# TorbenHellriegel/Speaker-Recognition-x-vectors

Measured on NVIDIA B200. Metric: x-vectors/sec, higher is better.
Workload: dtype bf16

## Files before the change

include/xvec_b200.h:

```cpp
#ifndef XVEC_B200_H_
#define XVEC_B200_H_

#include <stdint.h>

#ifdef __cplusplus
extern "C" {
#endif

#define XVEC_ABI_VERSION 7

#if defined(__GNUC__)
#define XVEC_API __attribute__((visibility("default")))
#else
#define XVEC_API
#endif

#define XVEC_F32 0
#define XVEC_BF16 1

#define XVEC_OK 0
#define XVEC_E_ARG (-1)
#define XVEC_E_CUDA (-2)
#define XVEC_E_DEVICE (-3)

#define XVEC_MAX_TAPS 8
#define XVEC_TILE_N 256
#define XVEC_POOL_BLOCK 128
#define XVEC_POOL_CHUNK 128
#define XVEC_MAX_STACK 6
#define XVEC_STACK_MAX_BANDS 512
#define XVEC_STACK_MAX_TAP_OFFSET 8

XVEC_API int xvec_abi_version(void);
XVEC_API const char* xvec_last_error(void);
XVEC_API int xvec_device_check(void);
XVEC_API int xvec_watchdog_code(void);
XVEC_API void xvec_watchdog_reset(void);

XVEC_API int xvec_debug_trace(long long* out_host, int n);

XVEC_API int64_t xvec_packed_k(int cin, int taps, int dtype);
XVEC_API int64_t xvec_packed_n(int n);

XVEC_API int xvec_pack_weight(const float* w_dev, int n, int taps, int cin, int dtype, void* out_dev, void* stream);

XVEC_API int xvec_tdnn_layer(const void* x_dev, int x_dtype, int64_t x_rows, int cin, int64_t x_ld,
                    const void* w_packed_dev, int n, const int32_t* tap_offsets_host, int taps,
                    const float* bias_dev, const float* bn_scale_dev, const float* bn_shift_dev, int relu,
                    void* y_dev, int y_dtype, int64_t y_ld, int64_t rows, void* splitk_ws_dev, int64_t splitk_ws_bytes,
                    void* stream);
XVEC_API int64_t xvec_splitk_workspace_bytes(int64_t rows, int cin, int taps, int n, int dtype);

XVEC_API int xvec_tdnn_pool_fused(const void* x_dev, int x_dtype, int64_t x_rows, int cin, int64_t x_ld,
                         const void* w_packed_dev, int n, const int32_t* tap_offsets_host, int taps,
                         const float* bias_dev, const int32_t* row_utt_dev, const int32_t* blk_slot_base_dev,
                         float* part_dev, int64_t rows, void* stream);

XVEC_API int xvec_build_layout(const int32_t* starts_dev, const int32_t* n_pool_dev, const int32_t* slot_start_dev, int n_utts,
                      int64_t rows, int32_t* row_utt_dev, int32_t* blk_slot_base_dev, void* stream);

XVEC_API int xvec_stats_pool_partial(const void* x_dev, int x_dtype, int64_t x_ld, int p, const int64_t* row_start_dev,
                            const int32_t* n_rows_dev, const int32_t* slot_start_dev, int n_utts, int max_chunks,
                            float* part_dev, float* pivot_dev, void* stream);

XVEC_API int xvec_pool_finalize(const float* part_dev, const int32_t* slot_start_dev, const int32_t* n_rows_dev, int n_utts,
                       int p, const float* bn_scale_dev, const float* bn_shift_dev, const float* pivot_dev, float* out_f32_dev,
                       void* out_lp_dev, int out_lp_dtype, int64_t out_lp_ld, void* stream);

typedef struct XvecLayerDesc {
  const void* w_packed_dev;
  const float* bias_dev;
  int32_t n;
  int32_t cin;
  int32_t taps;
  int32_t dtype;
  int32_t tap_offsets[XVEC_MAX_TAPS];
  const void* w_plain_dev;
} XvecLayerDesc;

XVEC_API int64_t xvec_stack_ctrl_bytes(int64_t rows, int n_tdnn);
XVEC_API int64_t xvec_stack_plan(int64_t rows, int n_layers, const int32_t* n_tiles_per_layer_host, int band, uint32_t* items_out_host,
                        int64_t capacity);
XVEC_API int xvec_tdnn_stack(const struct XvecLayerDesc* tdnn_host, int n_tdnn, const void* x_dev, int64_t rows, int64_t x_ld,
                    void* act0_dev, void* act1_dev, int64_t act_ld, const int32_t* row_utt_dev, const int32_t* blk_slot_base_dev,
                    float* part_dev, void* ctrl_dev, int64_t ctrl_bytes, int band, void* stream);

XVEC_API int xvec_linear_small(const void* x_dev, int dtype, int64_t rows, int k, int64_t x_ld, const void* w_dev, int n, int64_t w_ld,
                      const float* bias_dev, int relu, void* y_dev, int y_dtype, int64_t y_ld, void* stream);

XVEC_API int xvec_extract_forward(const XvecLayerDesc* tdnn_host, int n_tdnn, const void* x_dev, int64_t rows, int64_t x_ld,
                         void* act0_dev, void* act1_dev, int64_t act_ld, const int32_t* row_utt_dev,
                         const int32_t* blk_slot_base_dev, const int32_t* utt_slot_start_dev, const int32_t* n_pool_dev,
                         int n_utts, float* part_dev, const float* bn_last_scale_dev, const float* bn_last_shift_dev,
                         float* pooled_dev, void* pooled_lp_dev, const XvecLayerDesc* fc_host, int n_fc, void* fc_tmp_dev,
                         void* splitk_ws_dev, int64_t splitk_ws_bytes, float* out_dev, int64_t out_ld, void* ctrl_dev,
                         int64_t ctrl_bytes, void* stream);

XVEC_API int64_t xvec_mfcc_num_frames(int64_t n_samples);
XVEC_API int xvec_mfcc(const void* wav_dev, int wav_is_int16, const int64_t* wav_start_dev, const int32_t* wav_len_dev,
              const int64_t* row_start_dev, const int32_t* n_frames_dev, int n_utts, int max_frames,
              const float* norm_offset_dev, const float* norm_scale_dev, float* out_dev, int64_t out_ld, void* stream);
XVEC_API int xvec_wav_minmax(const void* wav_dev, int wav_is_int16, const int64_t* wav_start_dev, const int32_t* wav_len_dev,
                    int n_utts, float* norm_offset_dev, float* norm_scale_dev, void* stream);

XVEC_API int xvec_cast(const float* src_dev, int64_t src_ld, void* dst_dev, int dst_dtype, int64_t dst_ld, int64_t rows,
              int cols, void* stream);

XVEC_API int xvec_cosine_trials(const float* xvec_dev, int64_t ld, int dim, const float* mean_dev, const int32_t* enrol_dev,
                       const int32_t* test_dev, int64_t n_trials, float* out_dev, void* stream);

XVEC_API int xvec_split_tf32(const float* x_dev, int64_t ld, int64_t rows, int cols, float* out_dev, int64_t out_ld, void* stream);
XVEC_API int xvec_plda_rowterm(const float* x_dev, int64_t ld, int dim, const float* mean_dev, const float* y_dev, int64_t y_ld,
                      int64_t n, float* q_dev, void* stream);
XVEC_API int xvec_plda_trials(const float* x_dev, int64_t ld, int dim, const float* mean_dev, const float* p_dev, int64_t p_ld,
                     const float* q_dev, const int32_t* enrol_dev, const int32_t* test_dev, int64_t n_trials, float cst, float scale,
                     float* out_dev, void* stream);

#ifdef __cplusplus
}
#endif
#endif
```

speaker-recognition-x-vectors_b200/_lib.py:

```python
from __future__ import annotations

import ctypes
import os
import threading
from ctypes import POINTER, c_char_p, c_float, c_int, c_int32, c_int64, c_void_p

HERE = os.path.dirname(os.path.abspath(__file__))
LIB_PATH = os.environ.get("XVEC_LIB") or os.path.join(HERE, "libxvec_b200.so")

F32, BF16 = 0, 1
E_ARG, E_CUDA, E_DEVICE = -1, -2, -3
TILE_N, POOL_BLOCK, POOL_CHUNK, MAX_TAPS = 256, 128, 128, 8
ABI_VERSION = 7
MAX_STACK = 6
STACK_MAX_TAP_OFFSET = 8

class LayerDesc(ctypes.Structure):
    _fields_ = [("w_packed_dev", c_void_p), ("bias_dev", c_void_p), ("n", c_int32), ("cin", c_int32), ("taps", c_int32),
                ("dtype", c_int32), ("tap_offsets", c_int32 * MAX_TAPS), ("w_plain_dev", c_void_p)]


_SIGNATURES = {
    "xvec_abi_version": (c_int, []),
    "xvec_last_error": (c_char_p, []),
    "xvec_device_check": (c_int, []),
    "xvec_watchdog_code": (c_int, []),
    "xvec_watchdog_reset": (None, []),
    "xvec_debug_trace": (c_int, [c_void_p, c_int]),
    "xvec_packed_k": (c_int64, [c_int, c_int, c_int]),
    "xvec_packed_n": (c_int64, [c_int]),
    "xvec_pack_weight": (c_int, [c_void_p, c_int, c_int, c_int, c_int, c_void_p, c_void_p]),
    "xvec_tdnn_layer": (c_int, [c_void_p, c_int, c_int64, c_int, c_int64, c_void_p, c_int, POINTER(c_int32), c_int,
                                c_void_p, c_void_p, c_void_p, c_int, c_void_p, c_int, c_int64, c_int64, c_void_p, c_int64, c_void_p]),
    "xvec_splitk_workspace_bytes": (c_int64, [c_int64, c_int, c_int, c_int, c_int]),
    "xvec_tdnn_pool_fused": (c_int, [c_void_p, c_int, c_int64, c_int, c_int64, c_void_p, c_int, POINTER(c_int32), c_int,
                                     c_void_p, c_void_p, c_void_p, c_void_p, c_int64, c_void_p]),
    "xvec_build_layout": (c_int, [c_void_p, c_void_p, c_void_p, c_int, c_int64, c_void_p, c_void_p, c_void_p]),
    "xvec_stats_pool_partial": (c_int, [c_void_p, c_int, c_int64, c_int, c_void_p, c_void_p, c_void_p, c_int, c_int,
                                        c_void_p, c_void_p, c_void_p]),
    "xvec_pool_finalize": (c_int, [c_void_p, c_void_p, c_void_p, c_int, c_int, c_void_p, c_void_p, c_void_p, c_void_p, c_void_p,
                                   c_int, c_int64, c_void_p]),
    "xvec_extract_forward": (c_int, [POINTER(LayerDesc), c_int, c_void_p, c_int64, c_int64, c_void_p, c_void_p, c_int64, c_void_p, c_void_p,
                                     c_void_p, c_void_p, c_int, c_void_p, c_void_p, c_void_p, c_void_p, c_void_p, POINTER(LayerDesc), c_int,
                                     c_void_p, c_void_p, c_int64, c_void_p, c_int64, c_void_p, c_int64, c_void_p]),
    "xvec_stack_ctrl_bytes": (c_int64, [c_int64, c_int]),
    "xvec_stack_plan": (c_int64, [c_int64, c_int, POINTER(c_int32), c_int, c_void_p, c_int64]),
    "xvec_linear_small": (c_int, [c_void_p, c_int, c_int64, c_int, c_int64, c_void_p, c_int, c_int64, c_void_p, c_int, c_void_p, c_int, c_int64,
                                  c_void_p]),
    "xvec_tdnn_stack": (c_int, [POINTER(LayerDesc), c_int, c_void_p, c_int64, c_int64, c_void_p, c_void_p, c_int64, c_void_p, c_void_p,
                                c_void_p, c_void_p, c_int64, c_int, c_void_p]),
    "xvec_mfcc_num_frames": (c_int64, [c_int64]),
    "xvec_mfcc": (c_int, [c_void_p, c_int, c_void_p, c_void_p, c_void_p, c_void_p, c_int, c_int, c_void_p, c_void_p, c_void_p, c_int64, c_void_p]),
    "xvec_wav_minmax": (c_int, [c_void_p, c_int, c_void_p, c_void_p, c_int, c_void_p, c_void_p, c_void_p]),
    "xvec_cast": (c_int, [c_void_p, c_int64, c_void_p, c_int, c_int64, c_int64, c_int, c_void_p]),
    "xvec_cosine_trials": (c_int, [c_void_p, c_int64, c_int, c_void_p, c_void_p, c_void_p, c_int64, c_void_p, c_void_p]),
    "xvec_split_tf32": (c_int, [c_void_p, c_int64, c_int64, c_int, c_void_p, c_int64, c_void_p]),
    "xvec_plda_rowterm": (c_int, [c_void_p, c_int64, c_int, c_void_p, c_void_p, c_int64, c_int64, c_void_p, c_void_p]),
    "xvec_plda_trials": (c_int, [c_void_p, c_int64, c_int, c_void_p, c_void_p, c_int64, c_void_p, c_void_p, c_void_p, c_int64, c_float, c_float,
                                 c_void_p, c_void_p]),
}
EXPORTS = tuple(_SIGNATURES)

_lock = threading.Lock()
_lib = None


class XvecError(RuntimeError):
    def __init__(self, code: int, msg: str):
        super().__init__(f"libxvec_b200 error {code}: {msg}")
        self.code = code


def load(build_if_missing: bool = True) -> ctypes.CDLL:
    global _lib
    with _lock:
        if _lib is not None:
            return _lib
        if not os.path.exists(LIB_PATH):
            if not build_if_missing:
                raise ImportError(f"{LIB_PATH} is missing; run speaker-recognition-x-vectors_b200/build.py")
            from . import build as _build
            _build.build()
        lib = ctypes.CDLL(LIB_PATH)
        for name, (res, args) in _SIGNATURES.items():
            fn = getattr(lib, name)
            fn.restype = res
            fn.argtypes = args
        if lib.xvec_abi_version() != ABI_VERSION:
            raise ImportError(f"{LIB_PATH}: ABI {lib.xvec_abi_version()} != expected {ABI_VERSION}; rebuild")
        _lib = lib
        return lib


def check(rc: int) -> None:
    if rc != 0:
        raise XvecError(rc, load().xvec_last_error().decode("utf-8", "replace"))


def ptr(t) -> int | None:
    return None if t is None else t.data_ptr()


def stream_ptr(device_index: int | None = None) -> int:
    import torch
    return torch._C._cuda_getCurrentRawStream(torch.cuda.current_device() if device_index is None else device_index)


class on_device:
    __slots__ = ("ctx",)

    def __init__(self, device):
        import torch
        idx = device.index if device.index is not None else torch.cuda.current_device()
        self.ctx = None if idx == torch.cuda.current_device() else torch.cuda.device(idx)

    def __enter__(self):
        if self.ctx is not None:
            self.ctx.__enter__()

    def __exit__(self, *a):
        if self.ctx is not None:
            return self.ctx.__exit__(*a)


def dtype_code(torch_dtype) -> int:
    import torch
    if torch_dtype == torch.float32:
        return F32
    if torch_dtype == torch.bfloat16:
        return BF16
    raise ValueError(f"unsupported dtype {torch_dtype}; the kernels take float32 (TF32 math) or bfloat16")


def taps_array(offsets):
    arr = (c_int32 * len(offsets))(*[int(o) for o in offsets])
    return arr
```

speaker-recognition-x-vectors_b200/build.py:

```python
from __future__ import annotations

import os
import subprocess
import sys

HERE = os.path.dirname(os.path.abspath(__file__))
CSRC = os.path.join(HERE, "csrc")
LIB = os.path.join(HERE, "libxvec_b200.so")
SOURCES = ["capi.cu", "tdnn_gemm.cu", "tdnn_stack.cu", "fc_small.cu", "pool.cu", "mfcc.cu"]
HEADERS = ["ptx.cuh", "gemm_tile.cuh", "xvec_internal.h", os.path.join("..", "..", "include", "xvec_b200.h")]
NVCC_FLAGS = ["-gencode", "arch=compute_100a,code=sm_100a", "-O3", "-std=c++17", "-lineinfo", "-Xcompiler", "-fPIC",
              "-Xcompiler", "-fvisibility=hidden", "--expt-relaxed-constexpr"]


def _nvcc() -> str:
    for cand in (os.environ.get("NVCC"), "/usr/local/cuda/bin/nvcc", "nvcc"):
        if cand and (os.path.isabs(cand) and os.path.exists(cand) or not os.path.isabs(cand)):
            return cand
    raise RuntimeError("nvcc not found")


DEBUG_LIB = os.path.join(HERE, "libxvec_b200_debug.so")


def needs_build(lib: str = LIB) -> bool:
    if not os.path.exists(lib):
        return True
    t = os.path.getmtime(lib)
    deps = [os.path.join(CSRC, s) for s in SOURCES + HEADERS] + [os.path.abspath(__file__)]
    return any(os.path.getmtime(d) > t for d in deps)


def build(force: bool = False, verbose: bool = False, debug: bool = False) -> str:
    if debug:
        if not force and not needs_build(DEBUG_LIB):
            return DEBUG_LIB
        return _build_to(DEBUG_LIB, list(NVCC_FLAGS) + ["-DXVEC_DEBUG"], verbose, "_dbg")
    if not force and not needs_build():
        return LIB
    return _build_to(LIB, list(NVCC_FLAGS), verbose, "")


def _build_to(lib: str, flags, verbose: bool, suffix: str) -> str:
    flags = flags + (["-Xptxas", "-v"] if verbose else [])
    objs = []
    for s in SOURCES:
        obj = os.path.join(CSRC, s.replace(".cu", suffix + ".o"))
        cmd = [_nvcc()] + flags + ["-c", os.path.join(CSRC, s), "-o", obj]
        r = subprocess.run(cmd, capture_output=True, text=True)
        if verbose or r.returncode:
            sys.stderr.write(r.stdout + r.stderr)
        if r.returncode:
            raise RuntimeError(f"nvcc failed on {s}")
        objs.append(obj)
    cmd = [_nvcc(), "-shared", "-o", lib] + objs + ["-lcudart"]
    r = subprocess.run(cmd, capture_output=True, text=True)
    if r.returncode:
        sys.stderr.write(r.stdout + r.stderr)
        raise RuntimeError("link failed")
    return lib


if __name__ == "__main__":
    print(build(force="--force" in sys.argv, verbose="--verbose" in sys.argv, debug="--debug" in sys.argv))
```

speaker-recognition-x-vectors_b200/csrc/capi.cu:

```cuda
#include <stdarg.h>
#include <stdio.h>

#include "xvec_internal.h"

namespace xvec {

static thread_local char g_err[512] = "";

int set_error(int code, const char* fmt, ...) {
  va_list ap;
  va_start(ap, fmt);
  vsnprintf(g_err, sizeof(g_err), fmt, ap);
  va_end(ap);
  return code;
}

namespace {
struct DevInfo {
  int checked = 0;
  int sms = 0;
  int major = 0, minor = 0;
};
DevInfo g_dev[64];

DevInfo* cur_dev() {
  int d = 0;
  if (cudaGetDevice(&d) != cudaSuccess || d < 0 || d >= 64) return nullptr;
  DevInfo* di = &g_dev[d];
  if (!di->checked) {
    cudaDeviceProp prop;
    if (cudaGetDeviceProperties(&prop, d) != cudaSuccess) return nullptr;
    di->sms = prop.multiProcessorCount;
    di->major = prop.major;
    di->minor = prop.minor;
    di->checked = (prop.major == 10) ? 1 : -1;
  }
  return di;
}
}

int device_check() {
  DevInfo* di = cur_dev();
  if (!di) return set_error(XVEC_E_CUDA, "no usable CUDA device: %s", cudaGetErrorString(cudaGetLastError()));
  if (di->checked < 0)
    return set_error(XVEC_E_DEVICE, "device is sm_%d%d; these kernels are built for sm_100a only (no fallback)", di->major, di->minor);
  return XVEC_OK;
}

int num_sms() {
  DevInfo* di = cur_dev();
  return di ? di->sms : 1;
}

PFN_encodeTiled get_encode_tiled() {
  static const PFN_encodeTiled fn = [] {
    void* p = nullptr;
    cudaDriverEntryPointQueryResult qres;
    if (cudaGetDriverEntryPoint("cuTensorMapEncodeTiled", &p, cudaEnableDefault, &qres) == cudaSuccess &&
        qres == cudaDriverEntryPointSuccess)
      return reinterpret_cast<PFN_encodeTiled>(p);
    return static_cast<PFN_encodeTiled>(nullptr);
  }();
  return fn;
}

unsigned int* watchdog_host_word() {
  static std::mutex mu;
  static unsigned int* word = nullptr;
  std::lock_guard<std::mutex> lock(mu);
  if (!word) {
    void* p = nullptr;
    if (cudaHostAlloc(&p, 64, cudaHostAllocMapped | cudaHostAllocPortable) != cudaSuccess) return nullptr;
    word = static_cast<unsigned int*>(p);
    *word = 0u;
  }
  return word;
}

int read_watchdog() {
  unsigned int* w = watchdog_host_word();
  return w ? static_cast<int>(*reinterpret_cast<volatile unsigned int*>(w)) : 0;
}

int layer_desc(XvecLayerDesc* l, const void* w_packed, const float* bias, int n, int cin, int taps, int dtype, const int32_t* tap_offsets) {
  if (!tap_offsets) return set_error(XVEC_E_ARG, "tap_offsets_host is NULL");
  if (taps < 1 || taps > XVEC_MAX_TAPS) return set_error(XVEC_E_ARG, "taps must be in [1,%d]", XVEC_MAX_TAPS);
  *l = XvecLayerDesc{};
  l->w_packed_dev = w_packed;
  l->bias_dev = bias;
  l->n = n;
  l->cin = cin;
  l->taps = taps;
  l->dtype = dtype;
  for (int j = 0; j < taps; ++j) l->tap_offsets[j] = tap_offsets[j];
  return XVEC_OK;
}

}

using namespace xvec;

extern "C" {

int xvec_abi_version(void) { return XVEC_ABI_VERSION; }
const char* xvec_last_error(void) { return g_err; }
int xvec_device_check(void) { return device_check(); }
int xvec_watchdog_code(void) {
  cudaDeviceSynchronize();
  return read_watchdog();
}
void xvec_watchdog_reset(void) {
  if (unsigned int* w = watchdog_host_word()) *reinterpret_cast<volatile unsigned int*>(w) = 0u;
}

int xvec_debug_trace(long long* out_host, int n) { return read_trace(out_host, n); }

int64_t xvec_packed_k(int cin, int taps, int dtype) {
  const int kc = chunk_elems(dtype);
  return static_cast<int64_t>(taps) * ((cin + kc - 1) / kc) * kc;
}
int64_t xvec_splitk_workspace_bytes(int64_t rows, int cin, int taps, int n, int dtype) {
  if (rows <= 0 || cin <= 0 || taps < 1 || n <= 0) return 0;
  return splitk_workspace_bytes(rows, cin, taps, n, dtype);
}
int64_t xvec_packed_n(int n) { return static_cast<int64_t>((n + XVEC_TILE_N - 1) / XVEC_TILE_N) * XVEC_TILE_N; }

int xvec_tdnn_layer(const void* x_dev, int x_dtype, int64_t x_rows, int cin, int64_t x_ld, const void* w_packed_dev, int n,
                    const int32_t* tap_offsets_host, int taps, const float* bias_dev, const float* bn_scale_dev,
                    const float* bn_shift_dev, int relu, void* y_dev, int y_dtype, int64_t y_ld, int64_t rows, void* splitk_ws_dev,
                    int64_t splitk_ws_bytes, void* stream) {
  XvecLayerDesc l;
  const int rc = layer_desc(&l, w_packed_dev, bias_dev, n, cin, taps, x_dtype, tap_offsets_host);
  if (rc) return rc;
  return gemm_store(l, x_dev, x_rows, x_ld, rows, bn_scale_dev, bn_shift_dev, relu, y_dev, y_dtype, y_ld, splitk_ws_dev, splitk_ws_bytes,
                    stream);
}

int xvec_tdnn_pool_fused(const void* x_dev, int x_dtype, int64_t x_rows, int cin, int64_t x_ld, const void* w_packed_dev, int n,
                         const int32_t* tap_offsets_host, int taps, const float* bias_dev, const int32_t* row_utt_dev,
                         const int32_t* blk_slot_base_dev, float* part_dev, int64_t rows, void* stream) {
  XvecLayerDesc l;
  const int rc = layer_desc(&l, w_packed_dev, bias_dev, n, cin, taps, x_dtype, tap_offsets_host);
  if (rc) return rc;
  return gemm_pool(l, x_dev, x_rows, x_ld, rows, row_utt_dev, blk_slot_base_dev, part_dev, stream);
}

int64_t xvec_stack_ctrl_bytes(int64_t rows, int n_tdnn) { return stack_ctrl_bytes(rows, n_tdnn); }
int64_t xvec_stack_plan(int64_t rows, int n_layers, const int32_t* n_tiles_per_layer_host, int band, uint32_t* items_out_host,
                        int64_t capacity) {
  return stack_plan(rows, n_layers, n_tiles_per_layer_host, band, items_out_host, capacity);
}

int xvec_linear_small(const void* x_dev, int dtype, int64_t rows, int k, int64_t x_ld, const void* w_dev, int n, int64_t w_ld,
                      const float* bias_dev, int relu, void* y_dev, int y_dtype, int64_t y_ld, void* stream) {
  return fc_small_dispatch(x_dev, dtype, rows, k, x_ld, w_dev, n, w_ld, bias_dev, relu, y_dev, y_dtype, y_ld, stream);
}

int xvec_tdnn_stack(const XvecLayerDesc* tdnn, int n_tdnn, const void* x_dev, int64_t rows, int64_t x_ld, void* act0_dev, void* act1_dev,
                    int64_t act_ld, const int32_t* row_utt_dev, const int32_t* blk_slot_base_dev, float* part_dev, void* ctrl_dev,
                    int64_t ctrl_bytes, int band, void* stream) {
  if (!tdnn) return set_error(XVEC_E_ARG, "tdnn_host is NULL");
  return stack_dispatch(tdnn, n_tdnn, x_dev, rows, x_ld, act0_dev, act1_dev, act_ld, row_utt_dev, blk_slot_base_dev, part_dev, ctrl_dev,
                        ctrl_bytes, band, stream);
}

static int frame_stack(const XvecLayerDesc* tdnn, int n_tdnn, const void* x, int64_t rows, int64_t x_ld, void* act0, void* act1,
                       int64_t act_ld, const int32_t* row_utt, const int32_t* blk_slot_base, float* part, void* ctrl, int64_t ctrl_bytes,
                       void* stream) {
  if (ctrl && stack_supported(tdnn, n_tdnn, rows))
    return stack_dispatch(tdnn, n_tdnn, x, rows, x_ld, act0, act1, act_ld, row_utt, blk_slot_base, part, ctrl, ctrl_bytes, 0, stream);
  void* act[2] = {act0, act1};
  const void* h = x;
  int64_t h_ld = x_ld;
  for (int i = 0; i + 1 < n_tdnn; ++i) {
    const int rc = gemm_store(tdnn[i], h, rows, h_ld, rows, nullptr, nullptr, 1, act[i & 1], tdnn[i + 1].dtype, act_ld, nullptr, 0, stream);
    if (rc) return rc;
    h = act[i & 1];
    h_ld = act_ld;
  }
  return gemm_pool(tdnn[n_tdnn - 1], h, rows, h_ld, rows, row_utt, blk_slot_base, part, stream);
}

static int segment_head(const XvecLayerDesc* fc, int n_fc, const void* a, int64_t a_ld, int n_utts, void* fc_tmp, void* splitk_ws,
                        int64_t splitk_ws_bytes, float* out, int64_t out_ld, void* stream) {
  for (int i = 0; i < n_fc; ++i) {
    const XvecLayerDesc& l = fc[i];
    const bool final_layer = i == n_fc - 1;
    void* y = final_layer ? static_cast<void*>(out) : fc_tmp;
    const int y_dtype = final_layer ? XVEC_F32 : fc[i + 1].dtype;
    const int64_t y_ld = final_layer ? out_ld : l.n;
    const int relu = final_layer ? 0 : 1;
    int rc;
    if (l.w_plain_dev && fc_small_supported(n_utts, l.cin, l.n, a_ld, l.cin, a, l.w_plain_dev, l.dtype))
      rc = fc_small_dispatch(a, l.dtype, n_utts, l.cin, a_ld, l.w_plain_dev, l.n, l.cin, l.bias_dev, relu, y, y_dtype, y_ld, stream);
    else
      rc = gemm_store(l, a, n_utts, a_ld, n_utts, nullptr, nullptr, relu, y, y_dtype, y_ld, splitk_ws, splitk_ws_bytes, stream);
    if (rc) return rc;
    a = y;
    a_ld = y_ld;
  }
  return XVEC_OK;
}

int xvec_extract_forward(const XvecLayerDesc* tdnn, int n_tdnn, const void* x_dev, int64_t rows, int64_t x_ld, void* act0_dev,
                         void* act1_dev, int64_t act_ld, const int32_t* row_utt_dev, const int32_t* blk_slot_base_dev,
                         const int32_t* utt_slot_start_dev, const int32_t* n_pool_dev, int n_utts, float* part_dev,
                         const float* bn_last_scale_dev, const float* bn_last_shift_dev, float* pooled_dev, void* pooled_lp_dev,
                         const XvecLayerDesc* fc, int n_fc, void* fc_tmp_dev, void* splitk_ws_dev, int64_t splitk_ws_bytes,
                         float* out_dev, int64_t out_ld, void* ctrl_dev, int64_t ctrl_bytes, void* stream) {
  if (!tdnn || n_tdnn < 2 || n_fc < 0 || n_fc > 2 || (n_fc > 0 && !fc))
    return set_error(XVEC_E_ARG, "need >= 2 TDNN layers and 0 to 2 segment layers");
  if (!x_dev || !act0_dev || !act1_dev || !pooled_dev || (n_fc > 0 && !out_dev)) return set_error(XVEC_E_ARG, "null pointer argument");
  if (n_fc == 2 && !fc_tmp_dev) return set_error(XVEC_E_ARG, "fc_tmp_dev is NULL");
  const bool lp_head = n_fc > 0 && fc[0].dtype == XVEC_BF16;
  if (lp_head && !pooled_lp_dev) return set_error(XVEC_E_ARG, "pooled_lp_dev is required for bf16 segment layers");
  int rc = frame_stack(tdnn, n_tdnn, x_dev, rows, x_ld, act0_dev, act1_dev, act_ld, row_utt_dev, blk_slot_base_dev, part_dev, ctrl_dev,
                       ctrl_bytes, stream);
  if (rc) return rc;
  const int64_t pooled_ld = 2 * static_cast<int64_t>(tdnn[n_tdnn - 1].n);
  rc = xvec_pool_finalize(part_dev, utt_slot_start_dev, n_pool_dev, n_utts, tdnn[n_tdnn - 1].n, bn_last_scale_dev, bn_last_shift_dev, nullptr,
                          pooled_dev, pooled_lp_dev, XVEC_BF16, pooled_ld, stream);
  if (rc) return rc;
  return segment_head(fc, n_fc, lp_head ? pooled_lp_dev : static_cast<const void*>(pooled_dev), pooled_ld, n_utts, fc_tmp_dev, splitk_ws_dev,
                      splitk_ws_bytes, out_dev, out_ld, stream);
}

}
```

speaker-recognition-x-vectors_b200/csrc/pool.cu:

```cuda
#include <cuda_bf16.h>

#include "xvec_internal.h"

namespace xvec {

template <bool kBf16>
__global__ void __launch_bounds__(128)
stats_pool_partial_kernel(const void* __restrict__ x, long long ld, int p, const long long* __restrict__ row_start,
                          const int* __restrict__ n_rows, const int* __restrict__ slot_start, float* __restrict__ part,
                          float* __restrict__ pivot_out) {
  const int u = blockIdx.x;
  const int nr = n_rows[u];
  const int r0 = blockIdx.y * XVEC_POOL_CHUNK;
  if (r0 >= nr) return;
  const int r1 = min(nr, r0 + XVEC_POOL_CHUNK);
  const int c = (blockIdx.z * 128 + threadIdx.x) * 4;
  if (c >= p) return;
  const long long first = row_start[u] + r0;
  float s0 = 0.f, s1 = 0.f, s2 = 0.f, s3 = 0.f, q0 = 0.f, q1 = 0.f, q2 = 0.f, q3 = 0.f;
  float4 pv = make_float4(0.f, 0.f, 0.f, 0.f);
  auto acc = [&](float a, float b, float cc, float d) {
    a -= pv.x; b -= pv.y; cc -= pv.z; d -= pv.w;
    s0 += a; s1 += b; s2 += cc; s3 += d;
    q0 = fmaf(a, a, q0); q1 = fmaf(b, b, q1); q2 = fmaf(cc, cc, q2); q3 = fmaf(d, d, q3);
  };
  constexpr int U = 8;
  int r = r0;
  if constexpr (kBf16) {
    const uint2* src = reinterpret_cast<const uint2*>(reinterpret_cast<const __nv_bfloat16*>(x) + first * ld + c);
    const long long step = ld / 4;
    if (pivot_out) {
      const uint2 w = __ldg(reinterpret_cast<const uint2*>(reinterpret_cast<const __nv_bfloat16*>(x) + row_start[u] * ld + c));
      const float2 a = __bfloat1622float2(*reinterpret_cast<const __nv_bfloat162*>(&w.x));
      const float2 b = __bfloat1622float2(*reinterpret_cast<const __nv_bfloat162*>(&w.y));
      pv = make_float4(a.x, a.y, b.x, b.y);
    }
    for (; r + U <= r1; r += U) {
      uint2 v[U];
#pragma unroll
      for (int i = 0; i < U; ++i) v[i] = __ldcs(src + static_cast<long long>(r - r0 + i) * step);
#pragma unroll
      for (int i = 0; i < U; ++i) {
        const float2 a = __bfloat1622float2(*reinterpret_cast<const __nv_bfloat162*>(&v[i].x));
        const float2 b = __bfloat1622float2(*reinterpret_cast<const __nv_bfloat162*>(&v[i].y));
        acc(a.x, a.y, b.x, b.y);
      }
    }
    for (; r < r1; ++r) {
      const uint2 w = __ldcs(src + static_cast<long long>(r - r0) * step);
      const float2 a = __bfloat1622float2(*reinterpret_cast<const __nv_bfloat162*>(&w.x));
      const float2 b = __bfloat1622float2(*reinterpret_cast<const __nv_bfloat162*>(&w.y));
      acc(a.x, a.y, b.x, b.y);
    }
  } else {
    const float4* src = reinterpret_cast<const float4*>(reinterpret_cast<const float*>(x) + first * ld + c);
    const long long step = ld / 4;
    if (pivot_out) pv = __ldg(reinterpret_cast<const float4*>(reinterpret_cast<const float*>(x) + row_start[u] * ld + c));
    for (; r + U <= r1; r += U) {
      float4 v[U];
#pragma unroll
      for (int i = 0; i < U; ++i) v[i] = __ldcs(src + static_cast<long long>(r - r0 + i) * step);
#pragma unroll
      for (int i = 0; i < U; ++i) acc(v[i].x, v[i].y, v[i].z, v[i].w);
    }
    for (; r < r1; ++r) {
      const float4 w = __ldcs(src + static_cast<long long>(r - r0) * step);
      acc(w.x, w.y, w.z, w.w);
    }
  }
  if (pivot_out && blockIdx.y == 0) *reinterpret_cast<float4*>(pivot_out + static_cast<size_t>(u) * p + c) = pv;
  float* dst = part + static_cast<size_t>(slot_start[u] + blockIdx.y) * 2 * p + c;
  *reinterpret_cast<float4*>(dst) = make_float4(s0, s1, s2, s3);
  *reinterpret_cast<float4*>(dst + p) = make_float4(q0, q1, q2, q3);
}

__global__ void __launch_bounds__(128)
pool_finalize_kernel(const float* __restrict__ part, const int* __restrict__ slot_start, const int* __restrict__ n_rows, int p,
                     const float* __restrict__ scale, const float* __restrict__ shift, const float* __restrict__ pivot,
                     float* __restrict__ out, void* __restrict__ out_lp, int lp_dtype, long long lp_ld) {
  const int u = blockIdx.x;
  const int col = blockIdx.y * 128 + threadIdx.x;
  __shared__ double inv_n[2];
  if (threadIdx.x == 0) {
    const int n0 = n_rows[u];
    inv_n[0] = n0 > 0 ? 1.0 / n0 : 0.0;
    inv_n[1] = n0 > 1 ? 1.0 / (n0 - 1) : 0.0;
  }
  __syncthreads();
  if (col >= p) return;
  const int sl0 = slot_start[u], sl1 = slot_start[u + 1];
  double S = 0.0, Q = 0.0;
  int sl = sl0;
  for (; sl + 4 <= sl1; sl += 4) {
    float a[4], b[4];
#pragma unroll
    for (int i = 0; i < 4; ++i) {
      const float* src = part + static_cast<size_t>(sl + i) * 2 * p + col;
      a[i] = src[0];
      b[i] = src[p];
    }
#pragma unroll
    for (int i = 0; i < 4; ++i) {
      S += static_cast<double>(a[i]);
      Q += static_cast<double>(b[i]);
    }
  }
  for (; sl < sl1; ++sl) {
    const float* src = part + static_cast<size_t>(sl) * 2 * p + col;
    S += static_cast<double>(src[0]);
    Q += static_cast<double>(src[p]);
  }
  const int n = n_rows[u];
  const double nan = __longlong_as_double(0x7ff8000000000000LL);
  const double mean = n > 0 ? S * inv_n[0] + (pivot ? static_cast<double>(pivot[static_cast<size_t>(u) * p + col]) : 0.0) : nan;
  double var = n > 1 ? (Q - S * S * inv_n[0]) * inv_n[1] : nan;
  if (var < 0.0) var = 0.0;
  const float sc = scale ? scale[col] : 1.f;
  const float sh = shift ? shift[col] : 0.f;
  const float m = static_cast<float>(mean * sc + sh);
  const float sd = fabsf(sc) * sqrtf(static_cast<float>(var));
  out[static_cast<size_t>(u) * 2 * p + col] = m;
  out[static_cast<size_t>(u) * 2 * p + p + col] = sd;
  if (out_lp) {
    if (lp_dtype == XVEC_BF16) {
      __nv_bfloat16* o = reinterpret_cast<__nv_bfloat16*>(out_lp) + static_cast<size_t>(u) * lp_ld;
      o[col] = __float2bfloat16_rn(m);
      o[p + col] = __float2bfloat16_rn(sd);
    } else {
      float* o = reinterpret_cast<float*>(out_lp) + static_cast<size_t>(u) * lp_ld;
      o[col] = m;
      o[p + col] = sd;
    }
  }
}

__global__ void __launch_bounds__(256)
build_layout_kernel(const int* __restrict__ starts, const int* __restrict__ n_pool, const int* __restrict__ slot_start, int n_utts,
                    int rows, int n_blocks, int* __restrict__ row_utt, int* __restrict__ blk_slot_base) {
  const int i = blockIdx.x * blockDim.x + threadIdx.x;
  if (i < rows) {
    int lo = 0, hi = n_utts - 1;
    while (lo < hi) {
      const int mid = (lo + hi + 1) >> 1;
      if (starts[mid] <= i) lo = mid; else hi = mid - 1;
    }
    row_utt[i] = (i - starts[lo] < n_pool[lo]) ? lo : -1;
  }
  if (i < n_blocks) {
    const int first_row = i * XVEC_POOL_BLOCK;
    int lo = 0, hi = n_utts;
    while (lo < hi) {
      const int mid = (lo + hi) >> 1;
      if (starts[mid] + n_pool[mid] - 1 >= first_row) hi = mid; else lo = mid + 1;
    }
    int base = 0;
    if (lo < n_utts) {
      const int b0 = starts[lo] / XVEC_POOL_BLOCK;
      base = slot_start[lo] + (i > b0 ? i - b0 : 0);
    }
    blk_slot_base[i] = base;
  }
}

__global__ void cast_kernel(const float* __restrict__ src, long long src_ld, void* __restrict__ dst, int dst_dtype, long long dst_ld,
                            long long rows, int cols) {
  const long long total = rows * cols;
  for (long long i = blockIdx.x * static_cast<long long>(blockDim.x) + threadIdx.x; i < total;
       i += static_cast<long long>(gridDim.x) * blockDim.x) {
    const long long r = i / cols;
    const int c = static_cast<int>(i - r * cols);
    const float v = src[r * src_ld + c];
    if (dst_dtype == XVEC_BF16)
      reinterpret_cast<__nv_bfloat16*>(dst)[r * dst_ld + c] = __float2bfloat16_rn(v);
    else
      reinterpret_cast<float*>(dst)[r * dst_ld + c] = v;
  }
}

__global__ void pack_weight_kernel(const float* __restrict__ w, int n, int taps, int cin, int tap_k, long long n_pad, long long k_pad,
                                   int dtype, void* __restrict__ out) {
  const long long total = n_pad * k_pad;
  for (long long i = blockIdx.x * static_cast<long long>(blockDim.x) + threadIdx.x; i < total;
       i += static_cast<long long>(gridDim.x) * blockDim.x) {
    const long long row = i / k_pad;
    const int kk = static_cast<int>(i - row * k_pad);
    const int tap = kk / tap_k;
    const int ch = kk - tap * tap_k;
    const float v = (row < n && ch < cin) ? w[row * (static_cast<long long>(taps) * cin) + tap * cin + ch] : 0.f;
    const int bke = dtype == XVEC_BF16 ? 64 : 32;
    const long long o = (static_cast<long long>(kk / bke) * n_pad + row) * bke + kk % bke;
    if (dtype == XVEC_BF16)
      reinterpret_cast<__nv_bfloat16*>(out)[o] = __float2bfloat16_rn(v);
    else
      reinterpret_cast<float*>(out)[o] = v;
  }
}

__global__ void __launch_bounds__(256)
cosine_trials_kernel(const float* __restrict__ xv, long long ld, int dim, const float* __restrict__ mean, const int* __restrict__ enrol,
                     const int* __restrict__ test, long long n_trials, float* __restrict__ out) {
  const long long t = (blockIdx.x * static_cast<long long>(blockDim.x) + threadIdx.x) >> 5;
  const int lane = threadIdx.x & 31;
  if (t >= n_trials) return;
  const float* a = xv + static_cast<long long>(enrol[t]) * ld;
  const float* b = xv + static_cast<long long>(test[t]) * ld;
  float ab = 0.f, aa = 0.f, bb = 0.f;
  for (int i = lane; i < dim; i += 32) {
    const float mu = mean ? mean[i] : 0.f;
    const float x = a[i] - mu, y = b[i] - mu;
    ab = fmaf(x, y, ab);
    aa = fmaf(x, x, aa);
    bb = fmaf(y, y, bb);
  }
#pragma unroll
  for (int o = 16; o > 0; o >>= 1) {
    ab += __shfl_xor_sync(0xffffffffu, ab, o);
    aa += __shfl_xor_sync(0xffffffffu, aa, o);
    bb += __shfl_xor_sync(0xffffffffu, bb, o);
  }
  if (lane == 0) out[t] = ab * rsqrtf(aa) * rsqrtf(bb);
}

__global__ void split_tf32_kernel(const float* __restrict__ x, long long ld, long long rows, int cols, float* __restrict__ out, long long out_ld) {
  const long long total = rows * cols;
  for (long long i = blockIdx.x * static_cast<long long>(blockDim.x) + threadIdx.x; i < total;
       i += static_cast<long long>(gridDim.x) * blockDim.x) {
    const long long r = i / cols;
    const int c = static_cast<int>(i - r * cols);
    const float v = x[r * ld + c];
    const float hi = __uint_as_float(__float_as_uint(v) & 0xFFFFE000u);
    float* o = out + r * out_ld + c;
    o[0] = hi;
    o[cols] = v - hi;
    o[2 * cols] = hi;
  }
}
__global__ void __launch_bounds__(256)
plda_rowterm_kernel(const float* __restrict__ x, long long ld, int dim, const float* __restrict__ mean, const float* __restrict__ y,
                    long long y_ld, long long n, float* __restrict__ q) {
  const long long r = (blockIdx.x * static_cast<long long>(blockDim.x) + threadIdx.x) >> 5;
  const int lane = threadIdx.x & 31;
  if (r >= n) return;
  float acc = 0.f;
  for (int i = lane; i < dim; i += 32) acc = fmaf(x[r * ld + i] - mean[i], y[r * y_ld + i], acc);
#pragma unroll
  for (int o = 16; o > 0; o >>= 1) acc += __shfl_xor_sync(0xffffffffu, acc, o);
  if (lane == 0) q[r] = 0.5f * acc;
}
__global__ void __launch_bounds__(256)
plda_trials_kernel(const float* __restrict__ x, long long ld, int dim, const float* __restrict__ mean, const float* __restrict__ p,
                   long long p_ld, const float* __restrict__ q, const int* __restrict__ enrol, const int* __restrict__ test,
                   long long n_trials, float cst, float scale, float* __restrict__ out) {
  const long long t = (blockIdx.x * static_cast<long long>(blockDim.x) + threadIdx.x) >> 5;
  const int lane = threadIdx.x & 31;
  if (t >= n_trials) return;
  const int e = enrol[t], s = test[t];
  const float* pe = p + static_cast<long long>(e) * p_ld;
  const float* xs = x + static_cast<long long>(s) * ld;
  float acc = 0.f;
  for (int i = lane; i < dim; i += 32) acc = fmaf(pe[i], xs[i] - mean[i], acc);
#pragma unroll
  for (int o = 16; o > 0; o >>= 1) acc += __shfl_xor_sync(0xffffffffu, acc, o);
  if (lane == 0) out[t] = scale * (q[e] + q[s] + acc + cst);
}

static int grid_for(long long total) {
  const long long want = (total + 255) / 256;
  const long long cap = static_cast<long long>(num_sms()) * 16;
  return static_cast<int>(want < cap ? want : cap);
}

static int check_launch(const char* what) {
  cudaError_t e = cudaGetLastError();
  if (e != cudaSuccess) return set_error(XVEC_E_CUDA, "%s launch: %s", what, cudaGetErrorString(e));
  return XVEC_OK;
}

}

using namespace xvec;

extern "C" {

int xvec_build_layout(const int32_t* starts_dev, const int32_t* n_pool_dev, const int32_t* slot_start_dev, int n_utts, int64_t rows,
                      int32_t* row_utt_dev, int32_t* blk_slot_base_dev, void* stream) {
  int rc = device_check();
  if (rc) return rc;
  if (!starts_dev || !n_pool_dev || !slot_start_dev || !row_utt_dev || !blk_slot_base_dev) return set_error(XVEC_E_ARG, "null pointer argument");
  if (n_utts <= 0 || rows <= 0 || rows > 0x7fffff00LL) return set_error(XVEC_E_ARG, "bad n_utts / rows");
  const int n_blocks = static_cast<int>((rows + 255) / 256) * (256 / XVEC_POOL_BLOCK);
  const long long n = rows > n_blocks ? rows : n_blocks;
  build_layout_kernel<<<static_cast<unsigned>((n + 255) / 256), 256, 0, static_cast<cudaStream_t>(stream)>>>(
      starts_dev, n_pool_dev, slot_start_dev, n_utts, static_cast<int>(rows), n_blocks, row_utt_dev, blk_slot_base_dev);
  return check_launch("build_layout_kernel");
}

int xvec_stats_pool_partial(const void* x_dev, int x_dtype, int64_t x_ld, int p, const int64_t* row_start_dev,
                            const int32_t* n_rows_dev, const int32_t* slot_start_dev, int n_utts, int max_chunks, float* part_dev,
                            float* pivot_dev, void* stream) {
  int rc = device_check();
  if (rc) return rc;
  if (!x_dev || !row_start_dev || !n_rows_dev || !slot_start_dev || !part_dev) return set_error(XVEC_E_ARG, "null pointer argument");
  if (x_dtype != XVEC_F32 && x_dtype != XVEC_BF16) return set_error(XVEC_E_ARG, "bad x_dtype %d", x_dtype);
  if (p <= 0 || p % 4 != 0 || x_ld % 4 != 0 || x_ld < p) return set_error(XVEC_E_ARG, "p and x_ld must be positive multiples of 4, x_ld >= p");
  const int align = x_dtype == XVEC_BF16 ? 8 : 16;
  if ((reinterpret_cast<uintptr_t>(x_dev) % align) != 0 || (reinterpret_cast<uintptr_t>(part_dev) & 15u) != 0 ||
      (reinterpret_cast<uintptr_t>(pivot_dev) & 15u) != 0)
    return set_error(XVEC_E_ARG, "x_dev / part_dev / pivot_dev are not sufficiently aligned");
  if (n_utts <= 0 || max_chunks <= 0 || max_chunks > 65535) return set_error(XVEC_E_ARG, "bad n_utts / max_chunks");
  dim3 grid(n_utts, max_chunks, (p + 511) / 512);
  cudaStream_t st = static_cast<cudaStream_t>(stream);
  if (x_dtype == XVEC_BF16)
    stats_pool_partial_kernel<true><<<grid, 128, 0, st>>>(x_dev, x_ld, p, reinterpret_cast<const long long*>(row_start_dev), n_rows_dev,
                                                         slot_start_dev, part_dev, pivot_dev);
  else
    stats_pool_partial_kernel<false><<<grid, 128, 0, st>>>(x_dev, x_ld, p, reinterpret_cast<const long long*>(row_start_dev), n_rows_dev,
                                                          slot_start_dev, part_dev, pivot_dev);
  return check_launch("stats_pool_partial_kernel");
}

int xvec_pool_finalize(const float* part_dev, const int32_t* slot_start_dev, const int32_t* n_rows_dev, int n_utts, int p,
                       const float* bn_scale_dev, const float* bn_shift_dev, const float* pivot_dev, float* out_f32_dev, void* out_lp_dev,
                       int out_lp_dtype, int64_t out_lp_ld, void* stream) {
  int rc = device_check();
  if (rc) return rc;
  if (!part_dev || !slot_start_dev || !n_rows_dev || !out_f32_dev) return set_error(XVEC_E_ARG, "null pointer argument");
  if (n_utts <= 0 || p <= 0) return set_error(XVEC_E_ARG, "non-positive size");
  if ((bn_scale_dev == nullptr) != (bn_shift_dev == nullptr)) return set_error(XVEC_E_ARG, "bn_scale and bn_shift must be given together");
  if (out_lp_dev && (out_lp_dtype != XVEC_F32 && out_lp_dtype != XVEC_BF16)) return set_error(XVEC_E_ARG, "bad out_lp_dtype");
  if (out_lp_dev && out_lp_ld < 2 * p) return set_error(XVEC_E_ARG, "out_lp_ld < 2p");
  dim3 grid(n_utts, (p + 127) / 128);
  pool_finalize_kernel<<<grid, 128, 0, static_cast<cudaStream_t>(stream)>>>(part_dev, slot_start_dev, n_rows_dev, p, bn_scale_dev,
                                                                            bn_shift_dev, pivot_dev, out_f32_dev, out_lp_dev, out_lp_dtype,
                                                                            out_lp_ld);
  return check_launch("pool_finalize_kernel");
}

int xvec_cast(const float* src_dev, int64_t src_ld, void* dst_dev, int dst_dtype, int64_t dst_ld, int64_t rows, int cols, void* stream) {
  int rc = device_check();
  if (rc) return rc;
  if (!src_dev || !dst_dev) return set_error(XVEC_E_ARG, "null pointer argument");
  if (rows <= 0 || cols <= 0 || src_ld < cols || dst_ld < cols) return set_error(XVEC_E_ARG, "bad shape");
  if (dst_dtype != XVEC_F32 && dst_dtype != XVEC_BF16) return set_error(XVEC_E_ARG, "bad dst_dtype");
  const long long total = rows * cols;
  const int blocks = grid_for(total);
  cast_kernel<<<blocks, 256, 0, static_cast<cudaStream_t>(stream)>>>(src_dev, src_ld, dst_dev, dst_dtype, dst_ld, rows, cols);
  return check_launch("cast_kernel");
}

int xvec_pack_weight(const float* w_dev, int n, int taps, int cin, int dtype, void* out_dev, void* stream) {
  int rc = device_check();
  if (rc) return rc;
  if (!w_dev || !out_dev) return set_error(XVEC_E_ARG, "null pointer argument");
  if (n <= 0 || cin <= 0 || taps < 1 || taps > XVEC_MAX_TAPS) return set_error(XVEC_E_ARG, "bad shape");
  if (dtype != XVEC_F32 && dtype != XVEC_BF16) return set_error(XVEC_E_ARG, "bad dtype");
  const long long k_pad = xvec_packed_k(cin, taps, dtype);
  const long long n_pad = xvec_packed_n(n);
  const long long total = n_pad * k_pad;
  const int blocks = grid_for(total);
  pack_weight_kernel<<<blocks, 256, 0, static_cast<cudaStream_t>(stream)>>>(w_dev, n, taps, cin, static_cast<int>(k_pad / taps), n_pad,
                                                                           k_pad, dtype, out_dev);
  return check_launch("pack_weight_kernel");
}

int xvec_cosine_trials(const float* xvec_dev, int64_t ld, int dim, const float* mean_dev, const int32_t* enrol_dev,
                       const int32_t* test_dev, int64_t n_trials, float* out_dev, void* stream) {
  int rc = device_check();
  if (rc) return rc;
  if (!xvec_dev || !enrol_dev || !test_dev || !out_dev) return set_error(XVEC_E_ARG, "null pointer argument");
  if (dim <= 0 || ld < dim || n_trials <= 0) return set_error(XVEC_E_ARG, "bad shape");
  const long long blocks = (n_trials * 32 + 255) / 256;
  cosine_trials_kernel<<<static_cast<unsigned>(blocks), 256, 0, static_cast<cudaStream_t>(stream)>>>(xvec_dev, ld, dim, mean_dev, enrol_dev,
                                                                                                   test_dev, n_trials, out_dev);
  return check_launch("cosine_trials_kernel");
}

int xvec_split_tf32(const float* x_dev, int64_t ld, int64_t rows, int cols, float* out_dev, int64_t out_ld, void* stream) {
  int rc = device_check();
  if (rc) return rc;
  if (!x_dev || !out_dev) return set_error(XVEC_E_ARG, "null pointer argument");
  if (rows <= 0 || cols <= 0 || ld < cols || out_ld < 3 * static_cast<int64_t>(cols)) return set_error(XVEC_E_ARG, "bad shape");
  split_tf32_kernel<<<grid_for(rows * cols), 256, 0, static_cast<cudaStream_t>(stream)>>>(x_dev, ld, rows, cols, out_dev, out_ld);
  return check_launch("split_tf32_kernel");
}

int xvec_plda_rowterm(const float* x_dev, int64_t ld, int dim, const float* mean_dev, const float* y_dev, int64_t y_ld, int64_t n,
                      float* q_dev, void* stream) {
  int rc = device_check();
  if (rc) return rc;
  if (!x_dev || !mean_dev || !y_dev || !q_dev) return set_error(XVEC_E_ARG, "null pointer argument");
  if (dim <= 0 || ld < dim || y_ld < dim || n <= 0) return set_error(XVEC_E_ARG, "bad shape");
  const long long blocks = (n * 32 + 255) / 256;
  plda_rowterm_kernel<<<static_cast<unsigned>(blocks), 256, 0, static_cast<cudaStream_t>(stream)>>>(x_dev, ld, dim, mean_dev, y_dev, y_ld, n, q_dev);
  return check_launch("plda_rowterm_kernel");
}

int xvec_plda_trials(const float* x_dev, int64_t ld, int dim, const float* mean_dev, const float* p_dev, int64_t p_ld, const float* q_dev,
                     const int32_t* enrol_dev, const int32_t* test_dev, int64_t n_trials, float cst, float scale, float* out_dev,
                     void* stream) {
  int rc = device_check();
  if (rc) return rc;
  if (!x_dev || !mean_dev || !p_dev || !q_dev || !enrol_dev || !test_dev || !out_dev) return set_error(XVEC_E_ARG, "null pointer argument");
  if (dim <= 0 || ld < dim || p_ld < dim || n_trials <= 0) return set_error(XVEC_E_ARG, "bad shape");
  const long long blocks = (n_trials * 32 + 255) / 256;
  plda_trials_kernel<<<static_cast<unsigned>(blocks), 256, 0, static_cast<cudaStream_t>(stream)>>>(x_dev, ld, dim, mean_dev, p_dev, p_ld, q_dev,
                                                                                                 enrol_dev, test_dev, n_trials, cst, scale, out_dev);
  return check_launch("plda_trials_kernel");
}

}
```

speaker-recognition-x-vectors_b200/csrc/ptx.cuh:

```cuda
#pragma once
#include <cuda_runtime.h>
#include <cuda.h>
#include <stdint.h>

namespace xvec {

static __device__ unsigned int* g_watchdog_ptr = nullptr;

static __device__ __noinline__ void watchdog_report(unsigned int code) {
  unsigned int* p = g_watchdog_ptr;
  if (p) {
    *reinterpret_cast<volatile unsigned int*>(p) = code;
    __threadfence_system();
  }
}
static __device__ __noinline__ void watchdog_trip(unsigned int code) {
  watchdog_report(code);
  __trap();
}

__device__ __forceinline__ uint32_t smem_u32(const void* p) {
  return static_cast<uint32_t>(__cvta_generic_to_shared(p));
}

__device__ __forceinline__ bool elect_one() {
  uint32_t pred;
  asm volatile("{\n\t.reg .pred p;\n\telect.sync _|p, 0xffffffff;\n\tselp.u32 %0, 1, 0, p;\n\t}" : "=r"(pred));
  return pred != 0;
}

__device__ __forceinline__ void mbar_init(uint64_t* bar, uint32_t count) {
  asm volatile("mbarrier.init.shared::cta.b64 [%0], %1;" ::"r"(smem_u32(bar)), "r"(count) : "memory");
}
__device__ __forceinline__ void fence_mbar_init() {
  asm volatile("fence.mbarrier_init.release.cluster;" ::: "memory");
}
__device__ __forceinline__ void mbar_expect_tx(uint64_t* bar, uint32_t bytes) {
  asm volatile("mbarrier.arrive.expect_tx.shared::cta.b64 _, [%0], %1;" ::"r"(smem_u32(bar)), "r"(bytes) : "memory");
}
__device__ __forceinline__ void mbar_arrive(uint64_t* bar) {
  asm volatile("mbarrier.arrive.shared::cta.b64 _, [%0];" ::"r"(smem_u32(bar)) : "memory");
}
__device__ __forceinline__ bool mbar_try_wait(uint64_t* bar, uint32_t parity) {
  uint32_t done;
  asm volatile(
      "{\n\t.reg .pred p;\n\t"
      "mbarrier.try_wait.parity.shared::cta.b64 p, [%1], %2;\n\t"
      "selp.u32 %0, 1, 0, p;\n\t}"
      : "=r"(done)
      : "r"(smem_u32(bar)), "r"(parity)
      : "memory");
  return done != 0;
}
__device__ __forceinline__ bool mbar_test_wait(uint64_t* bar, uint32_t parity) {
  uint32_t done;
  asm volatile(
      "{\n\t.reg .pred p;\n\t"
      "mbarrier.test_wait.parity.shared::cta.b64 p, [%1], %2;\n\t"
      "selp.u32 %0, 1, 0, p;\n\t}"
      : "=r"(done)
      : "r"(smem_u32(bar)), "r"(parity)
      : "memory");
  return done != 0;
}
__device__ __forceinline__ void mbar_wait(uint64_t* bar, uint32_t parity, uint32_t code) {
  uint32_t spins = 0;
  while (!mbar_try_wait(bar, parity)) {
    if (++spins > (1u << 26)) {
      watchdog_trip(code);
    }
  }
}

__device__ __forceinline__ bool mbar_try_wait_a(uint32_t bar_addr, uint32_t parity) {
  uint32_t done;
  asm volatile(
      "{\n\t.reg .pred p;\n\t"
      "mbarrier.try_wait.parity.shared::cta.b64 p, [%1], %2;\n\t"
      "selp.u32 %0, 1, 0, p;\n\t}"
      : "=r"(done)
      : "r"(bar_addr), "r"(parity)
      : "memory");
  return done != 0;
}
__device__ __forceinline__ void mbar_wait_a(uint32_t bar_addr, uint32_t parity, uint32_t code) {
  uint32_t spins = 0;
  while (!mbar_try_wait_a(bar_addr, parity)) {
    if (++spins > (1u << 26)) watchdog_trip(code);
  }
}
__device__ __forceinline__ void mbar_expect_tx_a(uint32_t bar_addr, uint32_t bytes) {
  asm volatile("mbarrier.arrive.expect_tx.shared::cta.b64 _, [%0], %1;" ::"r"(bar_addr), "r"(bytes) : "memory");
}

__device__ __forceinline__ uint32_t mapa_u32(uint32_t smem_addr, uint32_t cta_rank) {
  uint32_t r;
  asm volatile("mapa.shared::cluster.u32 %0, %1, %2;" : "=r"(r) : "r"(smem_addr), "r"(cta_rank));
  return r;
}
__device__ __forceinline__ void mbar_arrive_cluster(uint32_t cluster_addr) {
  asm volatile("mbarrier.arrive.shared::cluster.b64 _, [%0];" ::"r"(cluster_addr) : "memory");
}
__device__ __forceinline__ uint32_t cluster_ctarank() {
  uint32_t r;
  asm volatile("mov.u32 %0, %%cluster_ctarank;" : "=r"(r));
  return r;
}
__device__ __forceinline__ void cluster_sync_all() {
  asm volatile("barrier.cluster.arrive.release.aligned;" ::: "memory");
  asm volatile("barrier.cluster.wait.acquire.aligned;" ::: "memory");
}

__device__ __forceinline__ void mbar_arrive_expect_tx_cluster(uint32_t cluster_addr, uint32_t bytes) {
  asm volatile("mbarrier.arrive.expect_tx.shared::cluster.b64 _, [%0], %1;" ::"r"(cluster_addr), "r"(bytes) : "memory");
}
__device__ __forceinline__ void st_async_cluster_u32(uint32_t cluster_addr, uint32_t v, uint32_t cluster_mbar) {
  asm volatile("st.async.weak.shared::cluster.mbarrier::complete_tx::bytes.u32 [%0], %1, [%2];" ::"r"(cluster_addr), "r"(v), "r"(cluster_mbar) : "memory");
}

__device__ __forceinline__ uint32_t ld_acquire_gpu_u32(const uint32_t* p) {
  uint32_t v;
  asm volatile("ld.acquire.gpu.global.u32 %0, [%1];" : "=r"(v) : "l"(p) : "memory");
  return v;
}
__device__ __forceinline__ void red_release_gpu_add_u32(uint32_t* p, uint32_t v) {
  asm volatile("red.release.gpu.global.add.u32 [%0], %1;" ::"l"(p), "r"(v) : "memory");
}
__device__ __forceinline__ uint32_t atom_add_acq_rel_cta_shared_u32(uint32_t smem_addr, uint32_t v) {
  uint32_t old;
  asm volatile("atom.acq_rel.cta.shared::cta.add.u32 %0, [%1], %2;" : "=r"(old) : "r"(smem_addr), "r"(v) : "memory");
  return old;
}
__device__ __forceinline__ void fence_proxy_async_global() { asm volatile("fence.proxy.async.global;" ::: "memory"); }

__device__ __forceinline__ void fence_proxy_async_smem() {
  asm volatile("fence.proxy.async.shared::cta;" ::: "memory");
}
__device__ __forceinline__ void tc_fence_before() { asm volatile("tcgen05.fence::before_thread_sync;" ::: "memory"); }
__device__ __forceinline__ void tc_fence_after() { asm volatile("tcgen05.fence::after_thread_sync;" ::: "memory"); }

__device__ __forceinline__ void tma_prefetch_desc(const CUtensorMap* m) {
  asm volatile("prefetch.tensormap [%0];" ::"l"(reinterpret_cast<uint64_t>(m)) : "memory");
}
__device__ __forceinline__ void tma_store_2d(const CUtensorMap* m, const void* smem_src, int32_t c0, int32_t c1, uint64_t l2_policy) {
  asm volatile("cp.async.bulk.tensor.2d.global.shared::cta.bulk_group.L2::cache_hint [%0, {%2, %3}], [%1], %4;"
               ::"l"(reinterpret_cast<uint64_t>(m)), "r"(smem_u32(smem_src)), "r"(c0), "r"(c1), "l"(l2_policy)
               : "memory");
}
constexpr uint64_t L2_EVICT_NORMAL = 0x1000000000000000ull;
constexpr uint64_t L2_EVICT_FIRST = 0x12F0000000000000ull;
constexpr uint64_t L2_EVICT_LAST = 0x14F0000000000000ull;
__device__ __forceinline__ void tma_store_commit() { asm volatile("cp.async.bulk.commit_group;" ::: "memory"); }
template <int kPending>
__device__ __forceinline__ void tma_store_wait_read() {
  asm volatile("cp.async.bulk.wait_group.read %0;" ::"n"(kPending) : "memory");
}
__device__ __forceinline__ void tma_store_wait_all() { asm volatile("cp.async.bulk.wait_group 0;" ::: "memory"); }
template <int kPending>
__device__ __forceinline__ void tma_store_wait_done() {
  asm volatile("cp.async.bulk.wait_group %0;" ::"n"(kPending) : "memory");
}

template <uint32_t kCols>
__device__ __forceinline__ void tmem_alloc_pair(uint32_t* smem_result) {
  asm volatile("tcgen05.alloc.cta_group::2.sync.aligned.shared::cta.b32 [%0], %1;" ::"r"(smem_u32(smem_result)), "n"(kCols) : "memory");
  asm volatile("tcgen05.relinquish_alloc_permit.cta_group::2.sync.aligned;" ::: "memory");
}
template <uint32_t kCols>
__device__ __forceinline__ void tmem_dealloc_pair(uint32_t taddr) {
  asm volatile("tcgen05.dealloc.cta_group::2.sync.aligned.b32 %0, %1;" ::"r"(taddr), "n"(kCols) : "memory");
}

__device__ __forceinline__ uint64_t umma_desc_sw128(uint32_t smem_addr) {
  return static_cast<uint64_t>((smem_addr & 0x3FFFFu) >> 4) | (1ull << 16) | (static_cast<uint64_t>(1024 >> 4) << 32) |
         (1ull << 46) | (2ull << 61);
}

__host__ __device__ constexpr uint32_t umma_idesc(uint32_t fmt, uint32_t m, uint32_t n) {
  return (1u << 4) | (fmt << 7) | (fmt << 10) | ((n >> 3) << 17) | ((m >> 4) << 24);
}

__device__ __forceinline__ uint32_t tma_step_pair(uint32_t elected, uint32_t is_leader, uint32_t full_bar_local, uint32_t full_bar_leader,
                                                  uint32_t tx_bytes, uint32_t smem_a, const CUtensorMap* map_a, int32_t a0, int32_t a1,
                                                  uint64_t pol_a, uint32_t smem_b, const CUtensorMap* map_b, int32_t b0, int32_t b1,
                                                  uint64_t pol_b, uint32_t probe_bar, uint32_t probe_par) {
  uint32_t rdy;
  asm volatile(
      "{\n\t"
      ".reg .pred pe, pl, pw;\n\t"
      "setp.ne.b32 pe, %1, 0;\n\t"
      "setp.ne.b32 pl, %2, 0;\n\t"
      "and.pred pl, pl, pe;\n\t"
      "@pl mbarrier.arrive.expect_tx.shared::cta.b64 _, [%3], %5;\n\t"
      "@pe cp.async.bulk.tensor.2d.cta_group::2.shared::cluster.global.mbarrier::complete_tx::bytes.L2::cache_hint [%6], [%7, {%8, %9}], [%4], %10;\n\t"
      "@pe cp.async.bulk.tensor.2d.cta_group::2.shared::cluster.global.mbarrier::complete_tx::bytes.L2::cache_hint [%11], [%12, {%13, %14}], [%4], %17;\n\t"
      "mbarrier.try_wait.parity.shared::cta.b64 pw, [%15], %16;\n\t"
      "selp.u32 %0, 1, 0, pw;\n\t"
      "}"
      : "=r"(rdy)
      : "r"(elected), "r"(is_leader), "r"(full_bar_local), "r"(full_bar_leader), "r"(tx_bytes), "r"(smem_a),
        "l"(reinterpret_cast<uint64_t>(map_a)), "r"(a0), "r"(a1), "l"(pol_a), "r"(smem_b), "l"(reinterpret_cast<uint64_t>(map_b)),
        "r"(b0), "r"(b1), "r"(probe_bar), "r"(probe_par), "l"(pol_b)
      : "memory");
  return rdy;
}

__device__ __forceinline__ uint32_t tma_step_one(uint32_t elected, uint32_t is_leader, uint32_t do_load, uint32_t bar_local, uint32_t bar_leader,
                                                 uint32_t tx, uint32_t smem_dst, const CUtensorMap* map, int32_t c0, int32_t c1, uint64_t pol,
                                                 uint32_t probe_bar, uint32_t probe_par) {
  uint32_t rdy;
  asm volatile(
      "{\n\t"
      ".reg .pred pe, pl, pw;\n\t"
      "setp.ne.b32 pe, %1, 0;\n\t"
      "setp.ne.b32 pl, %2, 0;\n\t"
      "and.pred pl, pl, pe;\n\t"
      "mbarrier.test_wait.parity.shared::cta.b64 pw, [%11], %12;\n\t"
      "@pl mbarrier.arrive.expect_tx.shared::cta.b64 _, [%3], %5;\n\t"
      "@pe cp.async.bulk.tensor.2d.cta_group::2.shared::cluster.global.mbarrier::complete_tx::bytes.L2::cache_hint [%6], [%7, {%8, %9}], [%4], %10;\n\t"
      "selp.u32 %0, 1, 0, pw;\n\t"
      "}"
      : "=r"(rdy)
      : "r"(elected & do_load), "r"(is_leader), "r"(bar_local), "r"(bar_leader), "r"(tx), "r"(smem_dst), "l"(reinterpret_cast<uint64_t>(map)),
        "r"(c0), "r"(c1), "l"(pol), "r"(probe_bar), "r"(probe_par)
      : "memory");
  return rdy;
}

__device__ __forceinline__ void tma_load_2d_pair(uint32_t bar_leader, uint32_t smem_dst, const CUtensorMap* map, int32_t c0, int32_t c1, uint64_t pol) {
  asm volatile(
      "cp.async.bulk.tensor.2d.cta_group::2.shared::cluster.global.mbarrier::complete_tx::bytes.L2::cache_hint [%0], [%1, {%2, %3}], [%4], %5;"
      ::"r"(smem_dst), "l"(reinterpret_cast<uint64_t>(map)), "r"(c0), "r"(c1), "r"(bar_leader), "l"(pol)
      : "memory");
}

enum { STEP_COMMIT_A = 1, STEP_COMMIT_B = 2, STEP_PROBE_A = 4, STEP_PROBE_B = 8 };
template <bool kTf32>
__device__ __forceinline__ uint32_t umma_step_pair(uint32_t elected, uint32_t tmem_d, uint64_t da, uint64_t db, uint32_t idesc,
                                                   uint32_t acc0, uint32_t flags, uint32_t commit_a_bar, uint32_t commit_b_bar,
                                                   uint32_t probe_a_bar, uint32_t probe_a_par, uint32_t probe_b_bar,
                                                   uint32_t probe_b_par) {
  uint32_t rdy;
#define XVEC_STEP_BODY(KIND)                                                                                      \
  asm volatile(                                                                                                   \
      "{\n\t"                                                                                                     \
      ".reg .pred pe, pacc, pt, pca, pcb, ppa, ppb, pwa, pwb;\n\t"                                                \
      ".reg .b64 a1, a2, a3, b1, b2, b3;\n\t"                                                                     \
      ".reg .b32 ra, rb, f;\n\t"                                                                                  \
      ".reg .b16 mk;\n\t"                                                                                         \
      "mov.b16 mk, 3;\n\t"                                                                                        \
      "setp.ne.b32 pe, %1, 0;\n\t"                                                                                \
      "setp.ne.b32 pacc, %6, 0;\n\t"                                                                              \
      "setp.eq.b32 pt, 0, 0;\n\t"                                                                                 \
      "and.b32 f, %7, 4;\n\tsetp.ne.b32 ppa, f, 0;\n\t"                                                          \
      "and.b32 f, %7, 8;\n\tsetp.ne.b32 ppb, f, 0;\n\t"                                                          \
      "setp.ne.b32 pwa, 0, 0;\n\t"                                                                                \
      "setp.ne.b32 pwb, 0, 0;\n\t"                                                                                \
      "@ppa mbarrier.test_wait.parity.shared::cta.b64 pwa, [%10], %11;\n\t"                                       \
      "@ppb mbarrier.test_wait.parity.shared::cta.b64 pwb, [%12], %13;\n\t"                                       \
      "add.u64 a1, %3, 2;\n\tadd.u64 a2, %3, 4;\n\tadd.u64 a3, %3, 6;\n\t"                                      \
      "add.u64 b1, %4, 2;\n\tadd.u64 b2, %4, 4;\n\tadd.u64 b3, %4, 6;\n\t"                                      \
      "@pe tcgen05.mma.cta_group::2.kind::" KIND " [%2], %3, %4, %5, pacc;\n\t"                                   \
      "@pe tcgen05.mma.cta_group::2.kind::" KIND " [%2], a1, b1, %5, pt;\n\t"                                     \
      "@pe tcgen05.mma.cta_group::2.kind::" KIND " [%2], a2, b2, %5, pt;\n\t"                                     \
      "@pe tcgen05.mma.cta_group::2.kind::" KIND " [%2], a3, b3, %5, pt;\n\t"                                     \
      "and.b32 f, %7, 2;\n\tsetp.ne.b32 pcb, f, 0;\n\tand.pred pcb, pcb, pe;\n\t"                               \
      "and.b32 f, %7, 1;\n\tsetp.ne.b32 pca, f, 0;\n\tand.pred pca, pca, pe;\n\t"                               \
      "@pcb tcgen05.commit.cta_group::2.mbarrier::arrive::one.shared::cluster.multicast::cluster.b64 [%9], mk;\n\t" \
      "@pca tcgen05.commit.cta_group::2.mbarrier::arrive::one.shared::cluster.multicast::cluster.b64 [%8], mk;\n\t" \
      "selp.u32 ra, 1, 0, pwa;\n\t"                                                                               \
      "selp.u32 rb, 2, 0, pwb;\n\t"                                                                               \
      "or.b32 %0, ra, rb;\n\t"                                                                                    \
      "}"                                                                                                         \
      : "=r"(rdy)                                                                                                 \
      : "r"(elected), "r"(tmem_d), "l"(da), "l"(db), "r"(idesc), "r"(acc0), "r"(flags), "r"(commit_a_bar),        \
        "r"(commit_b_bar), "r"(probe_a_bar), "r"(probe_a_par), "r"(probe_b_bar), "r"(probe_b_par)                 \
      : "memory")
  if constexpr (kTf32) {
    XVEC_STEP_BODY("tf32");
  } else {
    XVEC_STEP_BODY("f16");
  }
#undef XVEC_STEP_BODY
  return rdy;
}
template <bool kTf32, bool kLastTap>
__device__ __forceinline__ uint32_t umma_step_fixed(uint32_t elected, uint32_t tmem_d, uint32_t a_lo, uint32_t b_lo, uint32_t desc_hi, uint32_t idesc,
                                                    uint32_t acc0, uint32_t commit_a_bar, uint32_t commit_b_bar, uint32_t probe_a_bar,
                                                    uint32_t probe_a_par, uint32_t probe_b_bar, uint32_t probe_b_par) {
  uint32_t rdy;
#define XVEC_FIXED_BODY(KIND, PROBE_A, COMMIT_A)                                                                  \
  asm volatile(                                                                                                   \
      "{\n\t"                                                                                                     \
      ".reg .pred pe, pacc, pt, pwa, pwb;\n\t"                                                                    \
      ".reg .b64 a0, a1, a2, a3, b0, b1, b2, b3;\n\t"                                                             \
      ".reg .b32 ra, rb, t;\n\t"                                                                                  \
      ".reg .b16 mk;\n\t"                                                                                         \
      "mov.b16 mk, 3;\n\t"                                                                                        \
      "setp.ne.b32 pe, %13, 0;\n\t"                                                                               \
      "setp.ne.b32 pacc, %6, 0;\n\t"                                                                              \
      "setp.eq.b32 pt, 0, 0;\n\t"                                                                                 \
      "setp.ne.b32 pwa, 0, 0;\n\t"                                                                                \
      PROBE_A                                                                                                     \
      "mbarrier.test_wait.parity.shared::cta.b64 pwb, [%11], %12;\n\t"                                            \
      "mov.b64 a0, {%2, %4};\n\t"                                                                                 \
      "mov.b64 b0, {%3, %4};\n\t"                                                                                 \
      "add.u32 t, %2, 2;\n\tmov.b64 a1, {t, %4};\n\t"                                                            \
      "add.u32 t, %3, 2;\n\tmov.b64 b1, {t, %4};\n\t"                                                            \
      "add.u32 t, %2, 4;\n\tmov.b64 a2, {t, %4};\n\t"                                                            \
      "add.u32 t, %3, 4;\n\tmov.b64 b2, {t, %4};\n\t"                                                            \
      "add.u32 t, %2, 6;\n\tmov.b64 a3, {t, %4};\n\t"                                                            \
      "add.u32 t, %3, 6;\n\tmov.b64 b3, {t, %4};\n\t"                                                            \
      "@pe tcgen05.mma.cta_group::2.kind::" KIND " [%1], a0, b0, %5, pacc;\n\t"                                   \
      "@pe tcgen05.mma.cta_group::2.kind::" KIND " [%1], a1, b1, %5, pt;\n\t"                                     \
      "@pe tcgen05.mma.cta_group::2.kind::" KIND " [%1], a2, b2, %5, pt;\n\t"                                     \
      "@pe tcgen05.mma.cta_group::2.kind::" KIND " [%1], a3, b3, %5, pt;\n\t"                                     \
      "@pe tcgen05.commit.cta_group::2.mbarrier::arrive::one.shared::cluster.multicast::cluster.b64 [%8], mk;\n\t" \
      COMMIT_A                                                                                                    \
      "selp.u32 ra, 1, 0, pwa;\n\t"                                                                               \
      "selp.u32 rb, 2, 0, pwb;\n\t"                                                                               \
      "or.b32 %0, ra, rb;\n\t"                                                                                    \
      "}"                                                                                                         \
      : "=r"(rdy)                                                                                                 \
      : "r"(tmem_d), "r"(a_lo), "r"(b_lo), "r"(desc_hi), "r"(idesc), "r"(acc0), "r"(commit_a_bar), "r"(commit_b_bar),  \
        "r"(probe_a_bar), "r"(probe_a_par), "r"(probe_b_bar), "r"(probe_b_par), "r"(elected)                      \
      : "memory")
#define XVEC_FIXED_PROBE_A "mbarrier.test_wait.parity.shared::cta.b64 pwa, [%9], %10;\n\t"
#define XVEC_FIXED_COMMIT_A "@pe tcgen05.commit.cta_group::2.mbarrier::arrive::one.shared::cluster.multicast::cluster.b64 [%7], mk;\n\t"
  if constexpr (kTf32) {
    if constexpr (kLastTap) XVEC_FIXED_BODY("tf32", XVEC_FIXED_PROBE_A, XVEC_FIXED_COMMIT_A);
    else XVEC_FIXED_BODY("tf32", "", "");
  } else {
    if constexpr (kLastTap) XVEC_FIXED_BODY("f16", XVEC_FIXED_PROBE_A, XVEC_FIXED_COMMIT_A);
    else XVEC_FIXED_BODY("f16", "", "");
  }
#undef XVEC_FIXED_BODY
#undef XVEC_FIXED_PROBE_A
#undef XVEC_FIXED_COMMIT_A
  return rdy;
}
__device__ __forceinline__ void umma_commit_pair(uint64_t* bar, uint16_t cta_mask) {
  asm volatile("tcgen05.commit.cta_group::2.mbarrier::arrive::one.shared::cluster.multicast::cluster.b64 [%0], %1;"
               ::"r"(smem_u32(bar)), "h"(cta_mask) : "memory");
}
__device__ __forceinline__ void tmem_ld_32x32(uint32_t taddr, uint32_t (&v)[32]) {
  asm volatile(
      "tcgen05.ld.sync.aligned.32x32b.x32.b32 "
      "{%0, %1, %2, %3, %4, %5, %6, %7, %8, %9, %10, %11, %12, %13, %14, %15, "
      "%16, %17, %18, %19, %20, %21, %22, %23, %24, %25, %26, %27, %28, %29, %30, %31}, [%32];"
      : "=r"(v[0]), "=r"(v[1]), "=r"(v[2]), "=r"(v[3]), "=r"(v[4]), "=r"(v[5]), "=r"(v[6]), "=r"(v[7]), "=r"(v[8]),
        "=r"(v[9]), "=r"(v[10]), "=r"(v[11]), "=r"(v[12]), "=r"(v[13]), "=r"(v[14]), "=r"(v[15]), "=r"(v[16]),
        "=r"(v[17]), "=r"(v[18]), "=r"(v[19]), "=r"(v[20]), "=r"(v[21]), "=r"(v[22]), "=r"(v[23]), "=r"(v[24]),
        "=r"(v[25]), "=r"(v[26]), "=r"(v[27]), "=r"(v[28]), "=r"(v[29]), "=r"(v[30]), "=r"(v[31])
      : "r"(taddr)
      : "memory");
}
__device__ __forceinline__ void tmem_ld_wait() { asm volatile("tcgen05.wait::ld.sync.aligned;" ::: "memory"); }

}
```

speaker-recognition-x-vectors_b200/csrc/tdnn_stack.cu:

```cuda
#include "gemm_tile.cuh"
#include <cuda_bf16.h>

#include <mutex>
#include <type_traits>

namespace xvec {

template <bool kAllTf32>
struct StackCfg {
  static constexpr int SLOTS = 10;
  static constexpr int BOX_W = kAllTf32 ? 128 : 64;
  static constexpr int BOX_BYTES = 32 * BOX_W;
  static constexpr int NBUF = kAllTf32 ? 1 : 2;
  static constexpr int STAGE_BYTES = NBUF * BOX_BYTES;
};
constexpr int SLAB_ROWS_MAX = BM_CTA + XVEC_STACK_MAX_TAP_OFFSET;
constexpr int SLAB_BYTES = SLAB_ROWS_MAX * BK_BYTES;
constexpr int SLOT_BYTES = SLAB_BYTES;
static_assert(SLOT_BYTES % 1024 == 0 && SLOT_BYTES >= B_BYTES, "slot bases must stay 1024-byte aligned for SWIZZLE_128B and hold a weight tile");
constexpr int SCHED_SLOTS = 8;
constexpr int CREDIT_BARS = 4;
constexpr int STACK_RUNAHEAD = 1;
constexpr uint32_t ITEM_DONE = 0xFFFFFFFFu;
constexpr int SCHED_CONSUMERS = 2 * EPI_WARPS + 6;
static_assert((EPI_WARPS & (EPI_WARPS - 1)) == 0, "publish() counts the epilogue warps of a CTA modulo EPI_WARPS");
constexpr int DEP_WARP = 2 + EPI_WARPS;
constexpr int WPROD_WARP = DEP_WARP + 1;
constexpr int STACK_THREADS = GEMM_THREADS + 64;
constexpr int STACK_MAX_REGS = 112;

struct StackLayer {
  int n, n_tiles, taps, cpt;
  int tf32;
  int slab_rows;
  int n_pad;
  int tap_off[XVEC_MAX_TAPS];
  unsigned tap_off4;
  const float* bias;
};

struct StackMaps {
  CUtensorMap a[XVEC_MAX_STACK], b[XVEC_MAX_STACK], y[XVEC_MAX_STACK];
};

struct StackParams {
  int rows, m_tiles, n_layers;
  int band, n_bands;
  unsigned total_items;
  StackLayer L[XVEC_MAX_STACK];
  unsigned* counter;
  unsigned* ready;
  const int* row_utt;
  const int* blk_slot_base;
  float* part;
  unsigned long long pol_a, pol_b, pol_y;
  int dbg;
  int runahead;
  unsigned band_first[XVEC_STACK_MAX_BANDS + 1];
};

__host__ __device__ inline int band_layer_range(int band, int m_tiles, int b, int l, int* lo) {
  int a = b * band - l, z = (b + 1) * band - l;
  if (a < 0) a = 0;
  if (z > m_tiles) z = m_tiles;
  *lo = a;
  return z > a ? z - a : 0;
}
__host__ __device__ inline uint32_t decode_item(const StackParams& p, unsigned item, int& band_cursor) {
  while (item >= p.band_first[band_cursor + 1]) ++band_cursor;
  unsigned r = item - p.band_first[band_cursor];
  for (int l = 0; l < p.n_layers; ++l) {
    int lo;
    const unsigned nt = p.L[l].n_tiles;
    const unsigned cnt = band_layer_range(p.band, p.m_tiles, band_cursor, l, &lo) * nt;
    if (r < cnt) return static_cast<uint32_t>(l) | ((r % nt) << 3) | ((lo + r / nt) << 8);
    r -= cnt;
  }
  return ITEM_DONE;
}

#ifdef XVEC_DEBUG
#define XVEC_SDBG(p, bit) ((p).dbg & (bit))
#define XVEC_CNT(...) __VA_ARGS__
#else
#define XVEC_SDBG(p, bit) 0
#define XVEC_CNT(...)
#endif

template <int kSlots>
struct RingPos {
  int slot = 0;
  uint32_t ph = 0;
  __device__ __forceinline__ RingPos next() const {
    RingPos n = *this;
    if (++n.slot == kSlots) { n.slot = 0; n.ph ^= 1u; }
    return n;
  }
  __device__ __forceinline__ RingPos skip(int k) const {
    RingPos n = *this;
    n.slot += k;
    if (n.slot >= kSlots) { n.slot -= kSlots; n.ph ^= 1u; }
    return n;
  }
};

template <int kSlots>
struct MmaRing {
  RingPos<kSlots> pos;
  uint32_t rdy = 0;
};
struct TileK {
  int cpt, taps;
  uint32_t tap_off4;
  __device__ __forceinline__ explicit TileK(const StackLayer& L) : cpt(L.cpt), taps(L.taps), tap_off4(L.tap_off4) {}
};
static_assert(XVEC_MAX_TAPS <= 8 && XVEC_STACK_MAX_TAP_OFFSET < 16, "tap offsets are packed into 8 x 4 bits");

template <bool kTf32, int kSlots>
__device__ __forceinline__ void mma_tile(uint32_t ring_addr, uint32_t full_addr, uint32_t empty_addr, uint32_t d, const TileK k, MmaRing<kSlots>& r,
                                         bool swap_ab, unsigned long long& c_wait, unsigned long long& c_step) {
  constexpr uint32_t idesc = umma_idesc(kTf32 ? 2u : 1u, BM, BN);
  const uint64_t desc0 = umma_desc_sw128(ring_addr);
  uint32_t acc = 0;
  for (int ch = 0; ch < k.cpt; ++ch) {
    if (!(r.rdy & 1u)) {
      XVEC_CNT(const long long t0 = clock64();)
      mbar_wait_a(full_addr + 8u * r.pos.slot, r.pos.ph, 3);
      XVEC_CNT(c_wait += clock64() - t0;)
    }
    r.rdy &= ~1u;
    const int a_slot = r.pos.slot;
    r.pos = r.pos.next();
    const uint64_t slab_desc = desc0 + static_cast<uint32_t>(a_slot * (SLOT_BYTES >> 4));
    for (int tap = 0; tap < k.taps; ++tap) {
      if (!(r.rdy & 2u)) {
        XVEC_CNT(const long long t0 = clock64();)
        mbar_wait_a(full_addr + 8u * r.pos.slot, r.pos.ph, 3);
        XVEC_CNT(c_wait += clock64() - t0;)
      }
      tc_fence_after();
      const int b_slot = r.pos.slot;
      r.pos = r.pos.next();
      const uint64_t x_desc = slab_desc + ((k.tap_off4 >> (4 * tap)) & 15u) * (BK_BYTES >> 4);
      const uint64_t w_desc = desc0 + static_cast<uint32_t>(b_slot * (SLOT_BYTES >> 4));
      const uint64_t da = swap_ab ? w_desc : x_desc;
      const uint64_t db = swap_ab ? x_desc : w_desc;
      const bool last_tap = tap == k.taps - 1;
      const RingPos<kSlots> pa = r.pos;
      const RingPos<kSlots> pb = last_tap ? r.pos.next() : r.pos;
      const uint32_t flags = STEP_COMMIT_B | STEP_PROBE_B | (last_tap ? (STEP_COMMIT_A | STEP_PROBE_A) : 0u);
      XVEC_CNT(const long long ts = clock64();)
      const uint32_t got = umma_step_pair<kTf32>(elect_one() ? 1u : 0u, d, da, db, idesc, acc, flags, empty_addr + 8u * a_slot,
                                                 empty_addr + 8u * b_slot, full_addr + 8u * pa.slot, pa.ph, full_addr + 8u * pb.slot, pb.ph);
      XVEC_CNT(c_step += clock64() - ts;)
      r.rdy = (got & 2u) | (last_tap ? (got & 1u) : 0u);
      acc = 1u;
    }
  }
}

template <bool kTf32, int kSlots, int kTaps, bool kSwap>
__device__ __forceinline__ void mma_tile_fixed(uint32_t ring_addr, uint32_t full_addr, uint32_t empty_addr, uint32_t d, const TileK k,
                                               MmaRing<kSlots>& r, unsigned long long& c_wait, unsigned long long& c_step) {
  constexpr uint32_t idesc = umma_idesc(kTf32 ? 2u : 1u, BM, BN);
  const uint64_t desc0 = umma_desc_sw128(ring_addr);
  const uint32_t lo0 = static_cast<uint32_t>(desc0), hi = static_cast<uint32_t>(desc0 >> 32);
  const uint32_t elected = elect_one() ? 1u : 0u;
  uint32_t acc = 0;
#pragma unroll(kTaps == 1 ? 2 : 1)
  for (int ch = 0; ch < k.cpt; ++ch) {
    if (!(r.rdy & 1u)) {
      XVEC_CNT(const long long t0 = clock64();)
      mbar_wait_a(full_addr + 8u * r.pos.slot, r.pos.ph, 3);
      XVEC_CNT(c_wait += clock64() - t0;)
    }
    r.rdy &= ~1u;
    const int a_slot = r.pos.slot;
    r.pos = r.pos.next();
    const uint32_t slab_lo = lo0 + static_cast<uint32_t>(a_slot * (SLOT_BYTES >> 4));
    auto tap_step = [&](auto tap_c) {
      constexpr int tap = decltype(tap_c)::value;
      constexpr bool last_tap = tap == kTaps - 1;
      if (!(r.rdy & 2u)) {
        XVEC_CNT(const long long t0 = clock64();)
        mbar_wait_a(full_addr + 8u * r.pos.slot, r.pos.ph, 3);
        XVEC_CNT(c_wait += clock64() - t0;)
      }
      tc_fence_after();
      const int b_slot = r.pos.slot;
      r.pos = r.pos.next();
      const uint32_t x_lo = slab_lo + ((k.tap_off4 >> (4 * tap)) & 15u) * (BK_BYTES >> 4);
      const uint32_t w_lo = lo0 + static_cast<uint32_t>(b_slot * (SLOT_BYTES >> 4));
      const RingPos<kSlots> pa = r.pos;
      const RingPos<kSlots> pb = last_tap ? r.pos.next() : r.pos;
      XVEC_CNT(const long long ts = clock64();)
      const uint32_t got = umma_step_fixed<kTf32, last_tap>(elected, d, kSwap ? w_lo : x_lo, kSwap ? x_lo : w_lo, hi, idesc, acc,
                                                            empty_addr + 8u * a_slot, empty_addr + 8u * b_slot, full_addr + 8u * pa.slot, pa.ph,
                                                            full_addr + 8u * pb.slot, pb.ph);
      XVEC_CNT(c_step += clock64() - ts;)
      r.rdy = last_tap ? got : (got & 2u);
      acc = 1u;
    };
    static_assert(kTaps == 1 || kTaps == 3, "instantiated for the tap counts of the x-vector stack");
    tap_step(std::integral_constant<int, 0>{});
    if constexpr (kTaps == 3) {
      tap_step(std::integral_constant<int, 1>{});
      tap_step(std::integral_constant<int, 2>{});
    }
  }
}

template <bool kAllTf32>
constexpr int stack_smem_bytes() { return 1024 + StackCfg<kAllTf32>::SLOTS * SLOT_BYTES + EPI_WARPS * StackCfg<kAllTf32>::STAGE_BYTES; }
static_assert(stack_smem_bytes<false>() <= 227 * 1024 - 1024 && stack_smem_bytes<true>() <= 227 * 1024 - 1024,
              "operand ring + store staging (+ 1 KiB of static barriers) exceed the 227 KiB of shared memory a CTA can have");
constexpr int STACK_SMEM_LEFT_FOR_TAIL = 20 * 1024;
static_assert(228 * 1024 - stack_smem_bytes<false>() - 2048 - 2 * 1024 >= STACK_SMEM_LEFT_FOR_TAIL &&
              228 * 1024 - stack_smem_bytes<true>() - 2048 - 2 * 1024 >= STACK_SMEM_LEFT_FOR_TAIL,
              "the stack kernel must leave room on the SM for the tail kernels of the previous batch");

template <bool kAllTf32>
__global__ void __maxnreg__(STACK_MAX_REGS)
tdnn_stack_kernel(const __grid_constant__ StackMaps maps, const __grid_constant__ StackParams p) {
  extern __shared__ uint8_t smem_raw[];
  constexpr int RING_SLOTS = StackCfg<kAllTf32>::SLOTS;
  __shared__ uint64_t full_bar[RING_SLOTS], empty_bar[RING_SLOTS], tfull_bar[2], tempty_bar[2];
  __shared__ uint64_t sfull_bar[SCHED_SLOTS], sempty_bar[SCHED_SLOTS], dep_bar[SCHED_SLOTS], credit_bar[CREDIT_BARS];
  __shared__ uint32_t sched_item[SCHED_SLOTS];
  __shared__ uint32_t pub_cnt[4];
  __shared__ uint32_t tmem_base_smem;

  uint8_t* base = smem_raw + ((1024u - (smem_u32(smem_raw) & 1023u)) & 1023u);
  uint8_t* epi_smem = base + RING_SLOTS * SLOT_BYTES;

  const int warp = threadIdx.x >> 5;
  const int lane = threadIdx.x & 31;
  const uint32_t rank = cluster_ctarank();

  if (warp == 0 && lane == 0) {
    for (int c = 0; c < 4; ++c) pub_cnt[c] = 0;
    for (int l = 0; l < p.n_layers; ++l) {
      tma_prefetch_desc(&maps.a[l]);
      tma_prefetch_desc(&maps.b[l]);
      if (l + 1 < p.n_layers) tma_prefetch_desc(&maps.y[l]);
    }
    for (int s = 0; s < RING_SLOTS; ++s) {
      mbar_init(&full_bar[s], 1);
      mbar_init(&empty_bar[s], 1);
    }
    for (int b = 0; b < 2; ++b) {
      mbar_init(&tfull_bar[b], 1);
      mbar_init(&tempty_bar[b], 2 * EPI_WARPS);
    }
    for (int s = 0; s < SCHED_SLOTS; ++s) {
      mbar_init(&sfull_bar[s], 1);
      mbar_init(&sempty_bar[s], SCHED_CONSUMERS);
      mbar_init(&dep_bar[s], 1);
    }
    for (int c = 0; c < CREDIT_BARS; ++c) mbar_init(&credit_bar[c], 1);
    fence_mbar_init();
  }
  if (warp == 1) tmem_alloc_pair<TMEM_COLS>(&tmem_base_smem);
  tc_fence_before();
  __syncthreads();
  cluster_sync_all();
  tc_fence_after();
  const uint32_t tmem_base = tmem_base_smem;
  const uint32_t ring_addr = smem_u32(base), full_addr = smem_u32(full_bar), empty_addr = smem_u32(empty_bar);
  const uint32_t full_leader = mapa_u32(full_addr, 0);
  XVEC_CNT(long long dbg_c0 = clock64(); unsigned long long dbg_t0; asm volatile("mov.u64 %0, %%globaltimer;" : "=l"(dbg_t0));)

  auto ring_read = [&](int it) -> uint32_t {
    const int slot = it % SCHED_SLOTS;
    const uint32_t sph = (it / SCHED_SLOTS) & 1u;
    mbar_wait(&sfull_bar[slot], sph, 6);
    const uint32_t item = *reinterpret_cast<volatile uint32_t*>(&sched_item[slot]);
    __syncwarp();
    if (lane == 0) mbar_arrive_cluster(mapa_u32(smem_u32(&sempty_bar[slot]), 0));
    return item;
  };

  if (warp == 0 || warp == WPROD_WARP) {
    const bool slabs = warp == 0;
    static_assert(XVEC_MAX_TAPS + 1 <= StackCfg<kAllTf32>::SLOTS, "RingPos::skip wraps at most once");
    RingPos<RING_SLOTS> pos;
    uint32_t rdy = 0;
    XVEC_CNT(unsigned long long c_fw = 0, c_pub = 0;)
    for (int it = 0;; ++it) {
      XVEC_CNT(long long t0 = clock64();)
      const uint32_t item = ring_read(it);
      XVEC_CNT(c_pub += clock64() - t0; t0 = clock64();)
      if (item == ITEM_DONE) break;
      if (slabs) {
        mbar_wait(&dep_bar[it % SCHED_SLOTS], (it / SCHED_SLOTS) & 1u, 7);
        XVEC_CNT(c_fw += clock64() - t0;)
        if (rank == 0 && lane == 0) mbar_arrive(&credit_bar[it % CREDIT_BARS]);
      }
      const int layer = item & 7u, nt = (item >> 3) & 31u, mt = item >> 8;
      const StackLayer& L = p.L[layer];
      const int cpt = L.cpt, taps = L.taps, n_pad = L.n_pad;
      const uint32_t is_leader = rank == 0 ? 1u : 0u;
      if (slabs) {
        const int bke = (kAllTf32 || L.tf32) ? 32 : 64;
        const int m0 = mt * BM + static_cast<int>(rank) * BM_CTA;
        const CUtensorMap* ma = &maps.a[layer];
        const bool twice = XVEC_SDBG(p, 32);
        const uint32_t slab_tx = (twice ? 4u : 2u) * static_cast<uint32_t>(L.slab_rows) * BK_BYTES;
        const unsigned long long pol_a = p.pol_a;
        for (int ch = 0; ch < cpt; ++ch) {
          if (!rdy) mbar_wait_a(empty_addr + 8u * pos.slot, pos.ph ^ 1u, 1);
          const RingPos<RING_SLOTS> nxt = pos.skip(1 + taps);
          rdy = tma_step_one(elect_one() ? 1u : 0u, is_leader, 1u, full_addr + 8u * pos.slot, full_leader + 8u * pos.slot, slab_tx,
                             ring_addr + pos.slot * SLOT_BYTES, ma, ch * bke, m0, pol_a, empty_addr + 8u * nxt.slot, nxt.ph ^ 1u);
          if (twice && elect_one()) tma_load_2d_pair(full_leader + 8u * pos.slot, ring_addr + pos.slot * SLOT_BYTES, ma, ch * bke, m0, pol_a);
          pos = nxt;
        }
      } else {
        const int n0 = nt * BN + static_cast<int>(rank) * BN_CTA;
        const CUtensorMap* mb = &maps.b[layer];
        const unsigned long long pol_b = p.pol_b;
        for (int ch = 0; ch < cpt; ++ch) {
          RingPos<RING_SLOTS> pb = pos.next();
          int b_row = ch * n_pad + n0;
          for (int tap = 0; tap < taps; ++tap, b_row += cpt * n_pad) {
            if (!rdy) mbar_wait_a(empty_addr + 8u * pb.slot, pb.ph ^ 1u, 1);
            const RingPos<RING_SLOTS> nxt = tap == taps - 1 ? pb.skip(2) : pb.next();
            rdy = tma_step_one(elect_one() ? 1u : 0u, is_leader, 1u, full_addr + 8u * pb.slot, full_leader + 8u * pb.slot, 2u * B_BYTES,
                               ring_addr + pb.slot * SLOT_BYTES, mb, 0, b_row, pol_b, empty_addr + 8u * nxt.slot, nxt.ph ^ 1u);
            pb = nxt;
          }
          pos = pos.skip(1 + taps);
        }
      }
    }
    XVEC_CNT(if (slabs && lane == 0) {
      atomicAdd(p.counter + 3, static_cast<unsigned>(c_fw >> 6));
      atomicAdd(p.counter + 4, static_cast<unsigned>(c_pub >> 6));
    })
  } else if (warp == 1) {
    if (rank == 0) {
      MmaRing<RING_SLOTS> ring;
      unsigned long long c_full = 0, c_step = 0;
      XVEC_CNT(unsigned long long c_tempty = 0, c_ring = 0;)
      for (int it = 0;; ++it) {
        XVEC_CNT(const long long tr = clock64();)
        const uint32_t item = ring_read(it);
        XVEC_CNT(c_ring += clock64() - tr;)
        if (item == ITEM_DONE) break;
        XVEC_CNT(if (lane == 0) atomicAdd(p.counter + 32 + (item & 7u), static_cast<unsigned>((clock64() - tr) >> 4));)
        const StackLayer& L = p.L[item & 7u];
        const int buf = it & 1;
        const uint32_t use = (it >> 1) & 1;
        XVEC_CNT(const long long t0 = clock64();)
        mbar_wait(&tempty_bar[buf], use ^ 1u, 2);
        XVEC_CNT(c_tempty += clock64() - t0; const int dl = item & 7u; if (lane == 0) atomicAdd(p.counter + 16 + dl, static_cast<unsigned>((clock64() - t0) >> 4));)
        const uint32_t d = tmem_base + buf * BN;
        const bool pooled = static_cast<int>(item & 7u) == p.n_layers - 1;
        XVEC_CNT(const long long tk = clock64(); const unsigned long long full0 = c_full, step0 = c_step;)
        const TileK tk_(L);
        auto run = [&](auto tf_c) {
          constexpr bool tf = decltype(tf_c)::value;
          if (tk_.taps == 1) {
            if (pooled) mma_tile_fixed<tf, RING_SLOTS, 1, true>(ring_addr, full_addr, empty_addr, d, tk_, ring, c_full, c_step);
            else mma_tile_fixed<tf, RING_SLOTS, 1, false>(ring_addr, full_addr, empty_addr, d, tk_, ring, c_full, c_step);
          } else if (tk_.taps == 3) {
            if (pooled) mma_tile_fixed<tf, RING_SLOTS, 3, true>(ring_addr, full_addr, empty_addr, d, tk_, ring, c_full, c_step);
            else mma_tile_fixed<tf, RING_SLOTS, 3, false>(ring_addr, full_addr, empty_addr, d, tk_, ring, c_full, c_step);
          } else {
            mma_tile<tf, RING_SLOTS>(ring_addr, full_addr, empty_addr, d, tk_, ring, pooled, c_full, c_step);
          }
        };
        if constexpr (kAllTf32) {
          run(std::true_type{});
        } else {
          if (L.tf32) run(std::true_type{});
          else run(std::false_type{});
        }
        XVEC_CNT(if (lane == 0) {
          atomicAdd(p.counter + 40 + (item & 7u), static_cast<unsigned>((clock64() - tk) >> 4));
          atomicAdd(p.counter + 48 + (item & 7u), static_cast<unsigned>((c_full - full0) >> 4));
          atomicAdd(p.counter + 56 + (item & 7u), static_cast<unsigned>((c_step - step0) >> 4));
        })
        if (elect_one()) umma_commit_pair(&tfull_bar[buf], 0x3);
        __syncwarp();
        XVEC_CNT(if (lane == 0) atomicAdd(p.counter + 24 + (item & 7u), static_cast<unsigned>((clock64() - tr) >> 4));)
      }
      XVEC_CNT(if (lane == 0) {
        atomicAdd(p.counter + 5, static_cast<unsigned>(c_full >> 6));
        atomicAdd(p.counter + 6, static_cast<unsigned>(c_tempty >> 6));
        atomicAdd(p.counter + 10, static_cast<unsigned>(c_step >> 6));
        atomicAdd(p.counter + 11, static_cast<unsigned>(c_ring >> 6));
      })
    }
  } else if (warp == DEP_WARP) {
    XVEC_CNT(unsigned long long c_spun = 0, c_polls = 0;)
    int band_cursor = 0;
    unsigned raw_prev = 0;
    for (int it = 0;; ++it) {
      uint32_t item;
      if (rank == 0) {
        const int slot = it % SCHED_SLOTS;
        const uint32_t sph = (it / SCHED_SLOTS) & 1u;
        {
          const int depth = (raw_prev + static_cast<unsigned>(p.runahead + 1) * (gridDim.x >> 1) >= p.total_items) ? 1 : p.runahead;
          const int j = it - depth;
          if (j >= 0) mbar_wait(&credit_bar[j % CREDIT_BARS], static_cast<uint32_t>(j / CREDIT_BARS) & 1u, 8);
        }
        unsigned raw = 0;
        if (lane == 0) raw = atomicAdd(p.counter, 1u);
        raw = __shfl_sync(0xffffffffu, raw, 0);
        raw_prev = raw;
        item = raw < p.total_items ? decode_item(p, raw, band_cursor) : ITEM_DONE;
        mbar_wait(&sempty_bar[slot], sph ^ 1u, 5);
        if (lane == 0) {
          sched_item[slot] = item;
          mbar_arrive(&sfull_bar[slot]);
          const uint32_t peer_bar = mapa_u32(smem_u32(&sfull_bar[slot]), 1);
          mbar_arrive_expect_tx_cluster(peer_bar, 4);
          st_async_cluster_u32(mapa_u32(smem_u32(&sched_item[slot]), 1), item, peer_bar);
        }
        __syncwarp();
      } else {
        item = ring_read(it);
      }
      if (item == ITEM_DONE) break;
      const int layer = item & 7u, mt = item >> 8;
      if (layer > 0 && !XVEC_SDBG(p, 1)) {
        const unsigned target = static_cast<unsigned>(p.L[layer - 1].n_tiles) * 2u * EPI_WARPS;
        const int d = lane - 1;
        const bool mine = lane < 3 && mt + d >= 0 && mt + d < p.m_tiles && (d < 1 || rank == 1);
        const unsigned* f = p.ready + static_cast<size_t>(layer - 1) * p.m_tiles + (mine ? mt + d : mt);
        uint32_t spins = 0;
        while (__any_sync(0xffffffffu, mine && ld_acquire_gpu_u32(f) < target)) {
          if (++spins > (XVEC_SDBG(p, 8) ? (1u << 12) : (1u << 24))) {
            if (XVEC_SDBG(p, 16)) {
              watchdog_report(7u);
              break;
            }
            watchdog_trip(7u);
          }
        }
        XVEC_CNT(c_polls += spins; c_spun += spins ? 1 : 0;)
        if (!XVEC_SDBG(p, 4)) fence_proxy_async_global();
      }
      __syncwarp();
      if (lane == 0) mbar_arrive(&dep_bar[it % SCHED_SLOTS]);
    }
    XVEC_CNT(if (lane == 0) {
      atomicAdd(p.counter + 1, static_cast<unsigned>(c_spun));
      atomicAdd(p.counter + 2, static_cast<unsigned>(c_polls));
    })
  } else {
    const int q = warp & 3;
    const int cbeg = ((warp - 2) >> 2) * (BN / 2);
    uint8_t* out_stage = epi_smem + (warp - 2) * StackCfg<kAllTf32>::STAGE_BYTES;
    int store_seq = 0;
    constexpr int BOX_W = kAllTf32 ? 128 : 64;
    constexpr int BOX_BYTES = 32 * BOX_W;
    constexpr int NBUF = StackCfg<kAllTf32>::NBUF;
    constexpr int BOXES = (BN / 2) / 32;
    unsigned* pend = nullptr;
    int pend_it = 0;
    auto publish = [&](bool all) {
      if (lane == 0 && !XVEC_SDBG(p, 2)) {
        if (all) tma_store_wait_all();
        else tma_store_wait_done<BOXES>();
        if ((atom_add_acq_rel_cta_shared_u32(smem_u32(&pub_cnt[pend_it & 3]), 1u) & (EPI_WARPS - 1)) == EPI_WARPS - 1) {
          if (!XVEC_SDBG(p, 4)) fence_proxy_async_global();
          red_release_gpu_add_u32(pend, static_cast<uint32_t>(EPI_WARPS));
        }
      }
      pend = nullptr;
    };
    auto flush = [&]() { publish(true); };
    XVEC_CNT(unsigned long long e_wait[2] = {0, 0}, e_busy[2] = {0, 0}, e_tail = 0; long long e_t0 = 0, e_t1 = 0;)
    uint32_t item = ring_read(0);
    for (int it = 0;; ++it) {
      if (item == ITEM_DONE) break;
      const int layer = item & 7u, nt = (item >> 3) & 31u, mt = item >> 8;
      const StackLayer& L = p.L[layer];
      const int m0 = mt * BM + static_cast<int>(rank) * BM_CTA;
      const int n0 = nt * BN;
      const int buf = it & 1;
      const uint32_t use = (it >> 1) & 1;
      const bool pooled_tile = layer == p.n_layers - 1;
      const PoolArgs pa{p.rows, L.n, L.bias, p.row_utt, p.blk_slot_base, p.part};
      const int pch = n0 + static_cast<int>(rank) * BN_CTA + q * 32 + lane, pf0 = mt * BM + cbeg;
      PoolPrefetch pre{};
      if (pooled_tile) pre = pool_prefetch(pa, pch, pf0, lane);
      uint32_t next_item;
      {
        const int nslot = (it + 1) % SCHED_SLOTS;
        const uint32_t nph = ((it + 1) / SCHED_SLOTS) & 1u;
        if (pend && !mbar_test_wait(&sfull_bar[nslot], nph)) flush();
        next_item = ring_read(it + 1);
      }
      if (pend && !mbar_test_wait(&tfull_bar[buf], use)) flush();
      XVEC_CNT(e_t0 = clock64();)
      mbar_wait(&tfull_bar[buf], use, 4);
      tc_fence_after();
      XVEC_CNT(e_t1 = clock64(); e_wait[pooled_tile ? 0 : 1] += e_t1 - e_t0;)
      const uint32_t tbase = tmem_base + buf * BN + (static_cast<uint32_t>(q * 32) << 16);
      const int row0 = m0 + q * 32;
      bool released = false;
      auto release_tmem = [&]() {
        tc_fence_before();
        __syncwarp();
        if (lane == 0) mbar_arrive_cluster(mapa_u32(smem_u32(&tempty_bar[buf]), 0));
        released = true;
        XVEC_CNT(e_t0 = clock64(); e_busy[pooled_tile ? 0 : 1] += e_t0 - e_t1;)
      };

      if (XVEC_SDBG(p, 64)) {
        release_tmem();
        if (pend) flush();
        if (layer != p.n_layers - 1) {
          pend = p.ready + static_cast<size_t>(layer) * p.m_tiles + mt;
          pend_it = it;
        }
        item = next_item;
        continue;
      }
      if (pooled_tile) {
        pool_epilogue_tile_t(pa, pre, tmem_base + buf * BN + (static_cast<uint32_t>(q * 32) << 16) + cbeg, pch, pf0, lane, release_tmem);
        if (!released) release_tmem();
        if (pend) flush();
      } else {
        const CUtensorMap* my = &maps.y[layer];
        uint32_t va[32], vb[32];
        tmem_ld_32x32(tbase + cbeg, va);
        tmem_ld_wait();
#pragma unroll
        for (int k = 0; k < BOXES; ++k) {
          uint32_t(&v)[32] = (k & 1) ? vb : va;
          if (k + 1 < BOXES) tmem_ld_32x32(tbase + cbeg + 32 * (k + 1), (k & 1) ? va : vb);
          uint8_t* ob = out_stage + (store_seq % NBUF) * BOX_BYTES;
          const int col0 = n0 + cbeg + k * 32;
          float o[32];
          const float4* bp = reinterpret_cast<const float4*>(L.bias + col0);
#pragma unroll
          for (int j4 = 0; j4 < 32; j4 += 4) {
            const float4 bb = __ldg(bp + (j4 >> 2));
            const float2 a = __fadd2_rn(make_float2(__uint_as_float(v[j4 + 0]), __uint_as_float(v[j4 + 1])), make_float2(bb.x, bb.y));
            const float2 d = __fadd2_rn(make_float2(__uint_as_float(v[j4 + 2]), __uint_as_float(v[j4 + 3])), make_float2(bb.z, bb.w));
            o[j4 + 0] = a.x; o[j4 + 1] = a.y; o[j4 + 2] = d.x; o[j4 + 3] = d.y;
          }
          if (lane == 0) tma_store_wait_read<NBUF - 1>();
          __syncwarp();
          uint8_t* orow = ob + lane * BOX_W;
          if constexpr (!kAllTf32) {
#pragma unroll
            for (int j = 0; j < 4; ++j) {
              uint4 w;
              w.x = pack_bf16x2_relu(o[8 * j + 0], o[8 * j + 1]);
              w.y = pack_bf16x2_relu(o[8 * j + 2], o[8 * j + 3]);
              w.z = pack_bf16x2_relu(o[8 * j + 4], o[8 * j + 5]);
              w.w = pack_bf16x2_relu(o[8 * j + 6], o[8 * j + 7]);
              *reinterpret_cast<uint4*>(orow + ((j ^ ((lane >> 1) & 3)) << 4)) = w;
            }
          } else {
#pragma unroll
            for (int j = 0; j < 8; ++j) {
              const float4 w = make_float4(fmaxf(o[4 * j], 0.f), fmaxf(o[4 * j + 1], 0.f), fmaxf(o[4 * j + 2], 0.f), fmaxf(o[4 * j + 3], 0.f));
              *reinterpret_cast<float4*>(orow + ((j ^ (lane & 7)) << 4)) = w;
            }
          }
          if (k + 1 < BOXES) tmem_ld_wait();
          if (k == BOXES - 2) release_tmem();
          fence_proxy_async_smem();
          __syncwarp();
          if (lane == 0) {
            if (row0 < p.rows) tma_store_2d(my, ob, col0, row0, p.pol_y);
            tma_store_commit();
          }
          ++store_seq;
        }
        if (pend) publish(false);
        pend = p.ready + static_cast<size_t>(layer) * p.m_tiles + mt;
        pend_it = it;
      }
      XVEC_CNT(e_tail += clock64() - e_t0;)
      item = next_item;
    }
    XVEC_CNT(if (static_cast<int>(rank) == ((p.dbg >> 13) & 1) && warp == (((p.dbg >> 8) & 15) ? ((p.dbg >> 8) & 15) : 2) && lane == 0) {
      atomicAdd(p.counter + 12, static_cast<unsigned>(e_wait[0] >> 6));
      atomicAdd(p.counter + 13, static_cast<unsigned>(e_busy[0] >> 6));
      atomicAdd(p.counter + 14, static_cast<unsigned>(e_wait[1] >> 6));
      atomicAdd(p.counter + 15, static_cast<unsigned>(e_busy[1] >> 6));
      atomicAdd(p.counter + 7, static_cast<unsigned>(e_tail >> 6));
    })
    if (pend) flush();
    if (lane == 0) tma_store_wait_all();
  }

  tc_fence_before();
  __syncthreads();
  XVEC_CNT(if (blockIdx.x == 0 && threadIdx.x == 0) {
    unsigned long long t1;
    asm volatile("mov.u64 %0, %%globaltimer;" : "=l"(t1));
    p.counter[8] = static_cast<unsigned>((clock64() - dbg_c0) >> 6);
    p.counter[9] = static_cast<unsigned>(t1 - dbg_t0);
  })
  cluster_sync_all();
  if (warp == 1) {
    tc_fence_after();
    tmem_dealloc_pair<TMEM_COLS>(tmem_base);
  }
}

static int pick_band(int m_tiles, int n_layers, int pairs, int want) {
  int band = want;
  if (band <= 0) {
    const int target = (23 * pairs + 5) / 10, span = m_tiles + n_layers - 1;
    const int n_bands = span < target ? 1 : (span + target / 2) / target;
    band = (span + n_bands - 1) / n_bands;
  }
  if (band < n_layers) band = n_layers;
  while ((m_tiles + n_layers - 1 + band - 1) / band > XVEC_STACK_MAX_BANDS) band *= 2;
  return band;
}

static int fill_schedule(StackParams& p, int band) {
  p.band = band;
  p.n_bands = (p.m_tiles + p.n_layers - 1 + p.band - 1) / p.band;
  if (p.n_bands > XVEC_STACK_MAX_BANDS) return set_error(XVEC_E_ARG, "internal: too many bands");
  unsigned acc = 0;
  int64_t items_per_mtile = 0;
  for (int l = 0; l < p.n_layers; ++l) items_per_mtile += p.L[l].n_tiles;
  for (int b = 0; b < p.n_bands; ++b) {
    p.band_first[b] = acc;
    for (int l = 0; l < p.n_layers; ++l) {
      int lo;
      acc += static_cast<unsigned>(band_layer_range(p.band, p.m_tiles, b, l, &lo)) * p.L[l].n_tiles;
    }
  }
  p.band_first[p.n_bands] = acc;
  if (static_cast<int64_t>(acc) != items_per_mtile * p.m_tiles) return set_error(XVEC_E_ARG, "internal: band table does not cover the stack");
  p.total_items = acc;
  return XVEC_OK;
}

int64_t stack_plan(int64_t rows, int n_layers, const int32_t* n_tiles_per_layer, int band, uint32_t* items_out, int64_t capacity) {
  if (rows <= 0 || n_layers < 2 || n_layers > XVEC_MAX_STACK || !n_tiles_per_layer) return set_error(XVEC_E_ARG, "bad stack shape");
  static thread_local StackParams p;
  p = StackParams{};
  p.m_tiles = static_cast<int>((rows + BM - 1) / BM);
  p.n_layers = n_layers;
  for (int l = 0; l < n_layers; ++l) {
    if (n_tiles_per_layer[l] < 1 || n_tiles_per_layer[l] > 31) return set_error(XVEC_E_ARG, "bad n_tiles");
    p.L[l].n_tiles = n_tiles_per_layer[l];
  }
  int rc = fill_schedule(p, pick_band(p.m_tiles, n_layers, 74, band));
  if (rc) return rc;
  if (items_out) {
    int cursor = 0;
    for (unsigned i = 0; i < p.total_items && static_cast<int64_t>(i) < capacity; ++i) items_out[i] = decode_item(p, i, cursor);
  }
  return p.total_items;
}

int64_t stack_ctrl_bytes(int64_t rows, int n_layers) {
  if (rows <= 0 || n_layers < 2) return 0;
  const int64_t m_tiles = (rows + BM - 1) / BM;
  return 256 + (n_layers - 1) * m_tiles * 4;
}

XVEC_DEFINE_WATCHDOG_BINDER(bind_watchdog_stack)

bool stack_supported(const XvecLayerDesc* tdnn, int n_tdnn, int64_t rows) {
  if (n_tdnn < 2 || n_tdnn > XVEC_MAX_STACK || rows <= 0 || rows > 0x7fffff00LL) return false;
  if (tdnn[0].dtype != XVEC_F32 && tdnn[0].dtype != XVEC_BF16) return false;
  for (int i = 0; i < n_tdnn; ++i) {
    if (tdnn[i].taps < 1 || tdnn[i].taps > XVEC_MAX_TAPS) return false;
    if (i > 0 && (tdnn[i].dtype != tdnn[1].dtype || tdnn[i].cin != tdnn[i - 1].n)) return false;
    if (i + 1 < n_tdnn && (tdnn[i].n % BN != 0 || !tdnn[i].bias_dev)) return false;
    if ((tdnn[i].n + BN - 1) / BN > 31) return false;
    int max_off = 0;
    for (int j = 0; j < tdnn[i].taps; ++j) {
      if (tdnn[i].tap_offsets[j] < 0) return false;
      if (tdnn[i].tap_offsets[j] > max_off) max_off = tdnn[i].tap_offsets[j];
    }
    if (max_off > SLAB_ROWS_MAX - BM_CTA) return false;
  }
  return true;
}

struct StackKey {
  int dev, n_tdnn, band;
  int64_t rows, x_ld, act_ld;
  const void *x, *act0, *act1;
  XvecLayerDesc L[XVEC_MAX_STACK];
};
struct StackPlan {
  StackKey key;
  StackMaps maps;
  StackParams p;
  int grid;
  bool all_tf32;
  uint64_t stamp;
};
constexpr int STACK_PLAN_CACHE = 64;
static std::mutex g_plan_mu;
static StackPlan g_plans[STACK_PLAN_CACHE];
static uint64_t g_plan_clock = 0;

static int build_plan(StackPlan& pl, const XvecLayerDesc* tdnn, int n_tdnn, const void* x, int64_t rows, int64_t x_ld, void* act0, void* act1,
                      int64_t act_ld, int band) {
  pl.all_tf32 = tdnn[1].dtype == XVEC_F32;
  const int act_dtype = tdnn[1].dtype;
  StackMaps& maps = pl.maps;
  StackParams& p = pl.p;
  p = StackParams{};
  p.rows = static_cast<int>(rows);
  p.m_tiles = static_cast<int>((rows + BM - 1) / BM);
  p.n_layers = n_tdnn;
  void* act[2] = {act0, act1};
  const void* h = x;
  int64_t h_ld = x_ld;
  int h_dtype = tdnn[0].dtype;
  int rc;
  for (int l = 0; l < n_tdnn; ++l) {
    const XvecLayerDesc& d = tdnn[l];
    StackLayer& L = p.L[l];
    const int bke = chunk_elems(d.dtype);
    L.n = d.n;
    L.n_tiles = (d.n + BN - 1) / BN;
    L.taps = d.taps;
    L.cpt = (d.cin + bke - 1) / bke;
    L.tf32 = d.dtype == XVEC_F32 ? 1 : 0;
    int max_off = 0;
    for (int j = 0; j < d.taps; ++j) {
      L.tap_off[j] = d.tap_offsets[j];
      if (d.tap_offsets[j] > max_off) max_off = d.tap_offsets[j];
    }
    L.tap_off4 = 0;
    for (int j = 0; j < d.taps; ++j) L.tap_off4 |= static_cast<unsigned>(d.tap_offsets[j]) << (4 * j);
    L.slab_rows = BM_CTA + max_off;
    L.bias = d.bias_dev;
    if (reinterpret_cast<uintptr_t>(d.bias_dev) & 15u) return set_error(XVEC_E_ARG, "bias must be 16-byte aligned");
    const int64_t h_rows = window_rows(rows, d.cin, h_ld);
    if (h_rows < 0) return static_cast<int>(h_rows);
    rc = make_tmap_2d(&maps.a[l], h, h_dtype, static_cast<uint64_t>(d.cin), static_cast<uint64_t>(h_rows), static_cast<uint64_t>(h_ld),
                      bke, static_cast<uint32_t>(L.slab_rows));
    if (rc) return rc;
    L.n_pad = L.n_tiles * BN;
    rc = make_weight_tmap(&maps.b[l], d);
    if (rc) return rc;
    if (l + 1 < n_tdnn) {
      rc = make_tmap_2d(&maps.y[l], act[l & 1], act_dtype, static_cast<uint64_t>(d.n), static_cast<uint64_t>(rows),
                        static_cast<uint64_t>(act_ld), 32, 32, act_dtype == XVEC_BF16 ? CU_TENSOR_MAP_SWIZZLE_64B : CU_TENSOR_MAP_SWIZZLE_128B);
      if (rc) return rc;
      h = act[l & 1];
      h_ld = act_ld;
      h_dtype = act_dtype;
    } else {
      maps.y[l] = maps.a[l];
    }
  }
  for (int l = n_tdnn; l < XVEC_MAX_STACK; ++l) {
    maps.a[l] = maps.a[0];
    maps.b[l] = maps.b[0];
    maps.y[l] = maps.a[0];
  }
  const int max_pairs = num_sms() / 2;
  rc = fill_schedule(p, pick_band(p.m_tiles, n_tdnn, max_pairs, band));
  if (rc) return rc;
  l2_policies(&p.pol_a, &p.pol_b, &p.pol_y);
  p.runahead = STACK_RUNAHEAD;
  const int64_t pairs = static_cast<int64_t>(p.total_items) < max_pairs ? p.total_items : max_pairs;
  pl.grid = 2 * static_cast<int>(pairs);
  return XVEC_OK;
}

int stack_dispatch(const XvecLayerDesc* tdnn, int n_tdnn, const void* x, int64_t rows, int64_t x_ld, void* act0, void* act1,
                   int64_t act_ld, const int32_t* row_utt, const int32_t* blk_slot_base, float* part, void* ctrl, int64_t ctrl_bytes,
                   int band, void* stream) {
  int rc = device_check();
  if (rc) return rc;
  if (!stack_supported(tdnn, n_tdnn, rows)) return set_error(XVEC_E_ARG, "layer stack is not supported by the fused stack kernel");
  if (!x || !act0 || !act1 || !row_utt || !blk_slot_base || !part || !ctrl) return set_error(XVEC_E_ARG, "null pointer argument");
  if (ctrl_bytes < stack_ctrl_bytes(rows, n_tdnn) || (reinterpret_cast<uintptr_t>(ctrl) & 127u))
    return set_error(XVEC_E_ARG, "ctrl_dev must be 128-byte aligned and hold xvec_stack_ctrl_bytes() bytes");
  StackKey key;
  memset(&key, 0, sizeof(key));
  cudaGetDevice(&key.dev);
  key.n_tdnn = n_tdnn;
  key.band = band > 0 ? band : 0;
  key.rows = rows;
  key.x_ld = x_ld;
  key.act_ld = act_ld;
  key.x = x;
  key.act0 = act0;
  key.act1 = act1;
  for (int l = 0; l < n_tdnn; ++l) {
    rc = layer_desc(&key.L[l], tdnn[l].w_packed_dev, tdnn[l].bias_dev, tdnn[l].n, tdnn[l].cin, tdnn[l].taps, tdnn[l].dtype, tdnn[l].tap_offsets);
    if (rc) return rc;
  }
  StackMaps maps;
  StackParams p;
  int grid;
  bool all_tf32;
  {
    std::lock_guard<std::mutex> lock(g_plan_mu);
    StackPlan* hit = nullptr;
    StackPlan* victim = &g_plans[0];
    for (StackPlan& pl : g_plans) {
      if (pl.stamp && memcmp(&pl.key, &key, sizeof(key)) == 0) {
        hit = &pl;
        break;
      }
      if (pl.stamp < victim->stamp) victim = &pl;
    }
    if (!hit) {
      victim->stamp = 0;
      rc = build_plan(*victim, tdnn, n_tdnn, x, rows, x_ld, act0, act1, act_ld, band);
      if (rc) return rc;
      victim->key = key;
      hit = victim;
    }
    hit->stamp = ++g_plan_clock;
    maps = hit->maps;
    p = hit->p;
    grid = hit->grid;
    all_tf32 = hit->all_tf32;
  }
  p.counter = static_cast<unsigned*>(ctrl);
  p.ready = reinterpret_cast<unsigned*>(static_cast<char*>(ctrl) + 256);
  p.row_utt = row_utt;
  p.blk_slot_base = blk_slot_base;
  p.part = part;
#ifdef XVEC_DEBUG
  {
    const char* e = getenv("XVEC_STACK_DBG");
    p.dbg = e ? atoi(e) : 0;
  }
#endif
  cudaStream_t st = static_cast<cudaStream_t>(stream);
  cudaError_t e = cudaMemsetAsync(ctrl, 0, static_cast<size_t>(stack_ctrl_bytes(rows, n_tdnn)), st);
  if (e != cudaSuccess) return set_error(XVEC_E_CUDA, "cudaMemsetAsync(ctrl): %s", cudaGetErrorString(e));
  if (all_tf32)
    return launch_pair<tdnn_stack_kernel<true>>("tdnn_stack_kernel", STACK_THREADS, stack_smem_bytes<true>(), grid, bind_watchdog_stack, st, maps, p);
  return launch_pair<tdnn_stack_kernel<false>>("tdnn_stack_kernel", STACK_THREADS, stack_smem_bytes<false>(), grid, bind_watchdog_stack, st, maps, p);
}

}
```

speaker-recognition-x-vectors_b200/csrc/xvec_internal.h:

```cpp
#pragma once
#include <cuda.h>
#include <cuda_runtime.h>
#include <stdint.h>

#include <atomic>
#include <mutex>

#include "../../include/xvec_b200.h"

namespace xvec {

typedef CUresult (*PFN_encodeTiled)(CUtensorMap*, CUtensorMapDataType, cuuint32_t, void*, const cuuint64_t*, const cuuint64_t*,
                                    const cuuint32_t*, const cuuint32_t*, CUtensorMapInterleave, CUtensorMapSwizzle,
                                    CUtensorMapL2promotion, CUtensorMapFloatOOBfill);

int set_error(int code, const char* fmt, ...);
int device_check();
int num_sms();
PFN_encodeTiled get_encode_tiled();

inline int chunk_elems(int dtype) { return dtype == XVEC_F32 ? 32 : 64; }

int layer_desc(XvecLayerDesc* l, const void* w_packed, const float* bias, int n, int cin, int taps, int dtype, const int32_t* tap_offsets);
int gemm_store(const XvecLayerDesc& l, const void* x, int64_t x_rows, int64_t x_ld, int64_t rows, const float* bn_scale,
               const float* bn_shift, int relu, void* y, int y_dtype, int64_t y_ld, void* ws, int64_t ws_bytes, void* stream);
int gemm_pool(const XvecLayerDesc& l, const void* x, int64_t x_rows, int64_t x_ld, int64_t rows, const int32_t* row_utt,
              const int32_t* blk_slot_base, float* part, void* stream);
bool stack_supported(const XvecLayerDesc* tdnn, int n_tdnn, int64_t rows);
int64_t stack_ctrl_bytes(int64_t rows, int n_layers);
int64_t stack_plan(int64_t rows, int n_layers, const int32_t* n_tiles_per_layer, int band, uint32_t* items_out, int64_t capacity);
int stack_dispatch(const XvecLayerDesc* tdnn, int n_tdnn, const void* x, int64_t rows, int64_t x_ld, void* act0, void* act1,
                   int64_t act_ld, const int32_t* row_utt, const int32_t* blk_slot_base, float* part, void* ctrl, int64_t ctrl_bytes,
                   int band, void* stream);
bool fc_small_supported(int64_t rows, int k, int n, int64_t x_ld, int64_t w_ld, const void* x, const void* w, int dtype);
int fc_small_dispatch(const void* x, int dtype, int64_t rows, int k, int64_t x_ld, const void* w, int n, int64_t w_ld, const float* bias,
                      int relu, void* y, int y_dtype, int64_t y_ld, void* stream);
int64_t splitk_workspace_bytes(int64_t rows, int cin, int taps, int n, int dtype);

struct PerDeviceInit {
  std::mutex mu;
  std::atomic<bool> done[64];
  PerDeviceInit() {
    for (auto& d : done) d.store(false, std::memory_order_relaxed);
  }
};
template <class F>
inline int once_per_device(PerDeviceInit& s, F&& f) {
  int dev = -1;
  if (cudaGetDevice(&dev) != cudaSuccess || dev < 0 || dev >= 64) return f();
  if (s.done[dev].load(std::memory_order_acquire)) return XVEC_OK;
  std::lock_guard<std::mutex> lock(s.mu);
  if (!s.done[dev].load(std::memory_order_relaxed)) {
    const int rc = f();
    if (rc) return rc;
    s.done[dev].store(true, std::memory_order_release);
  }
  return XVEC_OK;
}

unsigned int* watchdog_host_word();
int read_watchdog();
int bind_watchdog_gemm();
int bind_watchdog_stack();
#define XVEC_DEFINE_WATCHDOG_BINDER(fn)                                                                               \
  int fn() {                                                                                                          \
    static PerDeviceInit once;                                                                                        \
    return once_per_device(once, [] {                                                                                 \
      unsigned int* w = watchdog_host_word();                                                                         \
      if (!w) return set_error(XVEC_E_CUDA, "cudaHostAlloc(watchdog word) failed");                                   \
      cudaError_t e = cudaMemcpyToSymbol(g_watchdog_ptr, &w, sizeof(w));                                              \
      if (e != cudaSuccess) return set_error(XVEC_E_CUDA, "cudaMemcpyToSymbol(watchdog): %s", cudaGetErrorString(e)); \
      return static_cast<int>(XVEC_OK);                                                                               \
    });                                                                                                               \
  }
int read_trace(long long* out_host, int n);

}
```

speaker-recognition-x-vectors_b200/xvector.py:

```python
from __future__ import annotations

from collections import OrderedDict

import numpy as np
import torch
import torch.nn as nn

from . import _lib, ops
from .layout import utterance_layout
from .tdnn_layer import TdnnLayer, _aligned_rows, tap_offsets

PRECISIONS = {"tf32": torch.float32, "fp32": torch.float32, "bf16": torch.bfloat16}


def _prep_fence(device, drain_all: bool):
    if device.type != "cuda":
        return
    with torch.cuda.device(device):
        if drain_all:
            torch.cuda.synchronize()
        else:
            torch.cuda.current_stream().synchronize()


class _Layout:

    def __init__(self, lengths, lost_frames, device, staging):
        starts, n_pool, slot_start, rows, n_slots = utterance_layout(lengths, lost_frames)
        self.rows, self.n_slots, self.n_utts = rows, n_slots, int(starts.shape[0])
        u = self.n_utts
        host = staging.get(3 * u + 1)
        host[:u] = torch.from_numpy(starts)
        host[u:2 * u] = torch.from_numpy(n_pool)
        host[2 * u:3 * u + 1] = torch.from_numpy(slot_start)
        dev = torch.empty(3 * u + 1, dtype=torch.int32, device=device)
        dev.copy_(host[: 3 * u + 1], non_blocking=True)
        staging.mark()
        self.starts, self.n_pool, self.utt_slot_start = dev[:u], dev[u:2 * u], dev[2 * u:]
        self.row_utt = torch.empty(rows, dtype=torch.int32, device=device)
        self.blk_slot_base = torch.empty(((rows + 255) // 256) * (256 // _lib.POOL_BLOCK), dtype=torch.int32, device=device)
        ops.build_layout_device(self.starts, self.n_pool, self.utt_slot_start, rows, self.row_utt, self.blk_slot_base)


class _PinnedStaging:

    RING = 16

    def __init__(self):
        self.bufs = [None] * self.RING
        self.evs = [None] * self.RING
        self.i = -1

    def get(self, n):
        self.i = (self.i + 1) % self.RING
        if self.evs[self.i] is not None:
            self.evs[self.i].synchronize()
        if self.bufs[self.i] is None or self.bufs[self.i].numel() < n:
            self.bufs[self.i] = torch.empty(max(n, 8192), dtype=torch.int32, pin_memory=True)
        return self.bufs[self.i]

    def mark(self):
        if self.evs[self.i] is None:
            self.evs[self.i] = torch.cuda.Event()
        self.evs[self.i].record()


class _Scratch:

    def __init__(self, device, act_dtype, widths, pool_dim):
        self.device, self.act_dtype, self.pool_dim = device, act_dtype, pool_dim
        per16 = 16 // torch.empty((), dtype=act_dtype).element_size()
        self.ld = (max(widths) + per16 - 1) // per16 * per16
        self.rows_cap = self.slots_cap = self.utts_cap = 0
        self.act = self.part = self.pooled = self.pooled_lp = self.ctrl = None
        self.fc_tmp = self.ws = self.ws_for = None

    def ensure(self, rows, n_slots, n_utts):
        if rows > self.rows_cap:
            self.rows_cap = max(rows, int(self.rows_cap * 1.25))
            self.act = [torch.empty((self.rows_cap, self.ld), dtype=self.act_dtype, device=self.device) for _ in range(2)]
            need = _lib.load().xvec_stack_ctrl_bytes(self.rows_cap, _lib.MAX_STACK)
            self.ctrl = torch.empty(need + 128, dtype=torch.uint8, device=self.device)
            off = (-self.ctrl.data_ptr()) % 128
            self.ctrl = self.ctrl[off: off + need]
        if n_slots > self.slots_cap:
            self.slots_cap = max(n_slots, int(self.slots_cap * 1.25))
            self.part = torch.empty((self.slots_cap, 2, self.pool_dim), dtype=torch.float32, device=self.device)
        if n_utts > self.utts_cap:
            self.utts_cap = max(n_utts, int(self.utts_cap * 1.25))
            self.pooled = torch.empty((self.utts_cap, 2 * self.pool_dim), dtype=torch.float32, device=self.device)
            self.pooled_lp = (torch.empty((self.utts_cap, 2 * self.pool_dim), dtype=self.act_dtype, device=self.device)
                              if self.act_dtype != torch.float32 else None)
            self.fc_tmp = None

    def ensure_head(self, n_utts, fc_shapes, width):
        if self.fc_tmp is None or self.fc_tmp.shape[0] < n_utts or self.fc_tmp.shape[1] != width:
            self.fc_tmp = torch.empty((max(n_utts, self.utts_cap), width), dtype=self.act_dtype, device=self.device)
        key = (n_utts, tuple(fc_shapes))
        if self.ws_for != key:
            lib = _lib.load()
            need = max(lib.xvec_splitk_workspace_bytes(n_utts, cin, 1, n, _lib.dtype_code(self.act_dtype)) for cin, n in fc_shapes)
            if need > 0 and (self.ws is None or self.ws.numel() < need):
                self.ws = torch.empty(need, dtype=torch.uint8, device=self.device)
            self.ws_for = key


class XVectorModel(nn.Module):
    def __init__(self, input_size=24, hidden_size=512, num_classes=1211, x_vector_size=512, x_vec_extract_layer=6,
                 batch_size=512, learning_rate=0.001, batch_norm=True, dropout_p=0.0, augmentations_per_sample=2,
                 data_folder_path="data", precision="tf32"):
        super().__init__()
        self.time_context_layers = nn.Sequential(
            TdnnLayer(input_size=input_size, output_size=hidden_size, context=[-2, -1, 0, 1, 2], batch_norm=batch_norm, dropout_p=dropout_p),
            TdnnLayer(input_size=hidden_size, output_size=hidden_size, context=[-2, 0, 2], batch_norm=batch_norm, dropout_p=dropout_p),
            TdnnLayer(input_size=hidden_size, output_size=hidden_size, context=[-3, 0, 3], batch_norm=batch_norm, dropout_p=dropout_p),
            TdnnLayer(input_size=hidden_size, output_size=hidden_size, batch_norm=batch_norm, dropout_p=dropout_p),
            TdnnLayer(input_size=hidden_size, output_size=1500, batch_norm=batch_norm, dropout_p=dropout_p),
        )
        self.segment_layer6 = nn.Linear(3000, x_vector_size)
        self.segment_layer7 = nn.Linear(x_vector_size, x_vector_size)
        self.output = nn.Linear(x_vector_size, num_classes)

        self.x_vec_extract_layer = x_vec_extract_layer
        self.batch_size = batch_size
        self.learning_rate = learning_rate
        self.input_size = input_size
        if precision not in PRECISIONS:
            raise ValueError(f"precision must be one of {sorted(PRECISIONS)}")
        self.precision = precision
        self._layouts: "OrderedDict[tuple, _Layout]" = OrderedDict()
        self._scratch = {}
        self._fc_prep = {}

    @property
    def act_dtype(self) -> torch.dtype:
        return PRECISIONS[self.precision]

    @property
    def lost_frames(self) -> int:
        return sum(tap_offsets(l.context)[-1] for l in self.time_context_layers)

    def _device(self):
        return self._modules["segment_layer6"]._parameters["weight"].device

    def _check_eval(self):
        if self.training:
            raise RuntimeError("xvec_b200.XVectorModel implements the eval-mode extraction path only; call .eval() first")

    def _layout_for(self, lengths) -> _Layout:
        lengths = np.asarray(lengths, dtype=np.int64)
        dev = self._device()
        key = (lengths.tobytes(), dev.index, _lib.stream_ptr(dev.index))
        lay = self._layouts.get(key)
        if lay is None:
            st = self._scratch.setdefault(("pin", str(dev)), _PinnedStaging())
            lay = _Layout(lengths, self.lost_frames, dev, st)
            self._layouts[key] = lay
            while len(self._layouts) > 128:
                self._layouts.popitem(last=False)
        else:
            self._layouts.move_to_end(key)
        return lay

    def _scratch_for(self, slot: int) -> _Scratch:
        dev = self._device()
        key = (dev.index, self.precision, slot)
        sc = self._scratch.get(key)
        if sc is None:
            layers = list(self.time_context_layers)
            sc = _Scratch(dev, self.act_dtype, [l.output_size for l in layers[:-1]], layers[-1].output_size)
            self._scratch[key] = sc
        return sc

    def _stack_kernel_ok(self) -> bool:
        layers = list(self.time_context_layers)
        return (2 <= len(layers) <= _lib.MAX_STACK
                and all(l.output_size % _lib.TILE_N == 0 for l in layers[:-1])
                and all(a.output_size == b.input_size for a, b in zip(layers[:-1], layers[1:]))
                and all(tap_offsets(l.context)[-1] <= _lib.STACK_MAX_TAP_OFFSET for l in layers))

    def _stack_params(self):
        layers = list(self.time_context_layers)
        fp = tuple(l._fingerprint() for l in layers) + (self.precision,)
        hit = self._fc_prep.get("stack")
        if hit is not None and hit[0] == fp:
            return hit[1]
        if hit is not None:
            _prep_fence(self._device(), drain_all=True)
        out, prev = [], None
        for i, layer in enumerate(layers):
            layer._check_eval()
            offs = tap_offsets(layer.context)
            W = layer.linear.weight.detach().double()
            b = (layer.linear.bias.detach().double() if layer.linear.bias is not None
                 else torch.zeros(layer.output_size, dtype=torch.float64, device=W.device))
            if prev is not None:
                s, h = prev
                b = b + W @ h.repeat(len(offs))
                W = W * s.repeat(len(offs))[None, :]
            dtype = torch.float32 if i == 0 else self.act_dtype
            out.append((ops.pack_weight(W.float(), len(offs), layer.input_size, dtype), ops.pad32(b.float()), offs))
            prev = layer.bn_affine64()
        last_bn = (None, None) if prev is None else (prev[0].float().contiguous(), prev[1].float().contiguous())
        res = (out, last_bn)
        self._fc_prep["stack"] = (fp, res)
        _prep_fence(self._device(), drain_all=False)
        return res

    def _pipeline(self):
        mods = self._modules
        layers = list(mods["time_context_layers"]._modules.values())
        use7 = self.x_vec_extract_layer == 7
        fcs = [mods["segment_layer6"], mods["segment_layer7"]] if use7 else [mods["segment_layer6"]]
        fp = (tuple(l._fingerprint() for l in layers), self.precision, use7,
              tuple((id(t), t._version) for f in fcs for t in f._parameters.values() if t is not None))
        hit = self._fc_prep.get("pipeline")
        if hit is not None and hit[0] == fp:
            return hit[1]
        if hit is not None:
            _prep_fence(self._device(), drain_all=True)
        stack, (scale5, shift5) = self._stack_params()
        code = _lib.dtype_code
        tdnn = (_lib.LayerDesc * len(layers))()
        window = None
        for i, (layer, (w, bias, offs)) in enumerate(zip(layers, stack)):
            d = tdnn[i]
            cin, taps = layer.input_size, len(offs)
            if i == 0 and list(offs) == list(range(taps)) and taps > 1 and (cin * 4) % 16 == 0 and self._stack_kernel_ok():
                w = ops.pack_weight(layer.linear.weight.detach().float(), 1, taps * cin, torch.float32)
                window = {"w": w, "cin": taps * cin}
                cin, offs = taps * cin, [0]
            d.w_packed_dev, d.bias_dev = w.data_ptr(), (bias.data_ptr() if bias is not None else None)
            d.n, d.cin, d.taps, d.dtype = layer.output_size, cin, len(offs), code(w.dtype)
            for j, o in enumerate(offs):
                d.tap_offsets[j] = o
        fc = (_lib.LayerDesc * len(fcs))()
        keep = []
        for i, lin in enumerate(fcs):
            w, b = self._fc(lin, self.act_dtype)
            keep.append((w, b))
            d = fc[i]
            d.w_packed_dev, d.bias_dev = w.data_ptr(), (b.data_ptr() if b is not None else None)
            d.n, d.cin, d.taps, d.dtype = lin.out_features, lin.in_features, 1, code(w.dtype)
            d.tap_offsets[0] = 0
            if lin.in_features % 8 == 0:
                w32 = lin.weight.detach().float().contiguous()
                w_plain = w32.clone() if self.act_dtype == torch.float32 else ops.cast(w32, self.act_dtype)
                keep.append(w_plain)
                d.w_plain_dev = w_plain.data_ptr()
        res = {"tdnn": tdnn, "n_tdnn": len(layers), "fc": fc, "n_fc": len(fcs), "keep": (stack, keep, scale5, shift5, window), "window": window,
               "scale5": scale5, "shift5": shift5, "out_dim": fcs[-1].out_features, "hidden": fcs[0].out_features,
               "fc_shapes": [(f.in_features, f.out_features) for f in fcs]}
        self._fc_prep["pipeline"] = (fp, res)
        _prep_fence(self._device(), drain_all=False)
        return res

    def _fc(self, lin: nn.Linear, dtype):
        fp = (id(lin.weight), lin.weight._version, id(lin.bias), lin.bias._version if lin.bias is not None else 0)
        hit = self._fc_prep.get((id(lin), dtype))
        if hit is not None and hit[0] == fp:
            return hit[1]
        if hit is not None:
            _prep_fence(lin.weight.device, drain_all=True)
        w = ops.pack_weight(lin.weight, 1, lin.in_features, dtype)
        b = ops.pad32(lin.bias)
        self._fc_prep[(id(lin), dtype)] = (fp, (w, b))
        _prep_fence(lin.weight.device, drain_all=False)
        return w, b

    def _linear(self, lin: nn.Linear, x2d: torch.Tensor, relu: bool, out_dtype) -> torch.Tensor:
        w, b = self._fc(lin, x2d.dtype)
        key = ("ws", x2d.shape[0], lin.in_features, lin.out_features, x2d.dtype, str(x2d.device), _lib.stream_ptr(x2d.device.index))
        if key not in self._fc_prep:
            self._fc_prep[key] = ops.splitk_workspace(x2d.shape[0], lin.in_features, 1, lin.out_features, x2d.dtype, x2d.device)
        return ops.tdnn_layer_flat(x2d, w, lin.out_features, [0], b, None, None, relu=relu, out_dtype=out_dtype, cin=lin.in_features,
                                   workspace=self._fc_prep[key])

    def _frames_for(self, flat_x: torch.Tensor, pipe) -> torch.Tensor:
        x = _aligned_rows(flat_x)
        if pipe["window"] is not None and x.stride(0) != self.input_size:
            x = _aligned_rows(x.contiguous())
        return x

    def _extract_forward(self, flat_x: torch.Tensor, lengths, slot: int, head: bool, out: torch.Tensor | None = None):
        self._check_eval()
        if not flat_x.is_cuda:
            raise ValueError("xvec_b200 has no CPU path: move the input (and the model) to a CUDA device")
        if flat_x.dim() != 2 or flat_x.shape[1] != self.input_size:
            raise ValueError(f"expected a flat (rows, {self.input_size}) frame matrix")
        lay = self._layout_for(lengths)
        if lay.rows != flat_x.shape[0]:
            raise ValueError("sum(lengths) does not match the number of rows")
        pipe = self._pipeline()
        sc = self._scratch_for(slot)
        sc.ensure(lay.rows, lay.n_slots, lay.n_utts)
        if flat_x.dtype != torch.float32:
            flat_x = flat_x.float()
        x = self._frames_for(flat_x, pipe)
        fc, n_fc, fc_tmp, ws = None, 0, None, None
        if head:
            sc.ensure_head(lay.n_utts, pipe["fc_shapes"], pipe["hidden"])
            fc, n_fc, fc_tmp, ws = pipe["fc"], pipe["n_fc"], sc.fc_tmp, sc.ws
            if out is None:
                out = torch.empty((lay.n_utts, pipe["out_dim"]), dtype=torch.float32, device=flat_x.device)
            elif (out.dtype != torch.float32 or out.device != flat_x.device or out.shape != (lay.n_utts, pipe["out_dim"]) or out.stride(1) != 1):
                raise ValueError(f"out must be a float32 ({lay.n_utts}, {pipe['out_dim']}) tensor on the input's device with unit column stride")
        lib = _lib.load()
        p = _lib.ptr
        with _lib.on_device(flat_x.device):
            _lib.check(lib.xvec_extract_forward(
                pipe["tdnn"], pipe["n_tdnn"], p(x), lay.rows, x.stride(0), p(sc.act[0]), p(sc.act[1]), sc.ld, p(lay.row_utt),
                p(lay.blk_slot_base), p(lay.utt_slot_start), p(lay.n_pool), lay.n_utts, p(sc.part), p(pipe["scale5"]), p(pipe["shift5"]),
                p(sc.pooled), p(sc.pooled_lp), fc, n_fc, p(fc_tmp), p(ws), 0 if ws is None else ws.numel(),
                p(out), 0 if out is None else out.stride(0), p(sc.ctrl), sc.ctrl.numel(), _lib.stream_ptr()))
        return lay, sc, out

    def pooled_stats_flat(self, flat_x: torch.Tensor, lengths, slot: int = 0) -> "tuple[torch.Tensor, torch.Tensor | None]":
        lay, sc, _ = self._extract_forward(flat_x, lengths, slot, head=False)
        return sc.pooled[: lay.n_utts], None if sc.pooled_lp is None else sc.pooled_lp[: lay.n_utts]

    def _head(self, pooled, pooled_lp, layer) -> torch.Tensor:
        a = pooled if pooled_lp is None else pooled_lp
        if layer == 7:
            h6 = self._linear(self.segment_layer6, a, relu=True, out_dtype=a.dtype)
            return self._linear(self.segment_layer7, h6, relu=False, out_dtype=torch.float32)
        return self._linear(self.segment_layer6, a, relu=False, out_dtype=torch.float32)

    def extract_x_vec_flat(self, flat_x: torch.Tensor, lengths, slot: int = 0, out: torch.Tensor | None = None) -> torch.Tensor:
        return self._extract_forward(flat_x, lengths, slot, head=True, out=out)[2]

    def extract_x_vec(self, x: torch.Tensor) -> torch.Tensor:
        if x.dim() != 3:
            raise ValueError(f"expected (B, T, {self.input_size}), got {tuple(x.shape)}")
        B, T, C = x.shape
        return self.extract_x_vec_flat(x.reshape(B * T, C), [T] * B)

    def forward(self, x: torch.Tensor) -> torch.Tensor:
        if x.dim() != 3:
            raise ValueError(f"expected (B, T, {self.input_size}), got {tuple(x.shape)}")
        B, T, C = x.shape
        pooled, pooled_lp = self.pooled_stats_flat(x.reshape(B * T, C), [T] * B)
        a = pooled if pooled_lp is None else pooled_lp
        h = self._linear(self.segment_layer6, a, relu=True, out_dtype=a.dtype)
        h = self._linear(self.segment_layer7, h, relu=True, out_dtype=a.dtype)
        return self._linear(self.output, h, relu=False, out_dtype=torch.float32)

    def stat_pool(self, x: torch.Tensor) -> torch.Tensor:
        if x.dim() != 3:
            raise ValueError("expected (B, T', P)")
        if not x.is_cuda:
            raise ValueError("xvec_b200 has no CPU path: move the input to a CUDA device")
        B, T, P = x.shape
        if x.dtype not in (torch.float32, torch.bfloat16):
            x = x.float()
        if x.stride(2) != 1 or x.stride(0) != T * x.stride(1) or P % 4 or x.stride(1) % 4 or x.data_ptr() % 16:
            x = x.contiguous()
            if P % 4:
                raise ValueError("stat_pool needs a channel count that is a multiple of 4")
        ld = x.stride(1)
        flat = torch.as_strided(x, (B * T, P), (ld, 1))
        return ops.stats_pool_ragged(flat, np.arange(B, dtype=np.int64) * T, np.full(B, T, dtype=np.int32))

    def test_step(self, batch, batch_index=0):
        samples, labels, ids = batch
        x_vecs = self.extract_x_vec(samples.float())
        return [(x_vecs, labels, ids)]

    def load_reference_checkpoint(self, path: str, map_location="cpu", trust_pickle: bool = False):
        try:
            ckpt = torch.load(path, map_location=map_location, weights_only=True)
        except Exception as e:
            if not trust_pickle:
                raise RuntimeError(f"{path} cannot be read with weights_only=True ({type(e).__name__}: {e}); pass trust_pickle=True "
                                   "only for a checkpoint from a trusted source") from e
            ckpt = torch.load(path, map_location=map_location, weights_only=False)
        sd = ckpt.get("state_dict", ckpt) if isinstance(ckpt, dict) else ckpt
        own = self.state_dict()
        missing = [k for k in own if k not in sd and not k.endswith("num_batches_tracked")]
        if missing:
            raise KeyError(f"checkpoint lacks {len(missing)} parameter(s) of the x-vector model, e.g. {missing[:3]}")
        return self.load_state_dict({k: v for k, v in sd.items() if k in own}, strict=False)
```

Baseline: 914,000.

## Fuse pooling finalize into persistent TDNN stack kernel via dedicated finalize warp

Adds a finalize warp to the persistent fused TDNN stack kernel. Epilogue warps publish the utterance ranges they have just pooled into a shared-memory queue, and per-utterance arrival counters in the ctrl buffer track completed groups. Once all groups for an utterance have arrived, the finalize warp computes mean/std, applies batch norm, and writes both the fp32 and bf16 pooled outputs. This removes the separate pool_finalize launch and overlaps finalization with the GEMM tail, at the cost of extra threads and shared memory per CTA, more ctrl memory, and added synchronisation complexity.

```diff
diff --git a/include/xvec_b200.h b/include/xvec_b200.h
--- a/include/xvec_b200.h
+++ b/include/xvec_b200.h
@@ -7,7 +7,7 @@
 extern "C" {
 #endif
 
-#define XVEC_ABI_VERSION 7
+#define XVEC_ABI_VERSION 8
 
 #if defined(__GNUC__)
 #define XVEC_API __attribute__((visibility("default")))
@@ -78,7 +78,7 @@
   const void* w_plain_dev;
 } XvecLayerDesc;
 
-XVEC_API int64_t xvec_stack_ctrl_bytes(int64_t rows, int n_tdnn);
+XVEC_API int64_t xvec_stack_ctrl_bytes(int64_t rows, int n_tdnn, int n_utts);
 XVEC_API int64_t xvec_stack_plan(int64_t rows, int n_layers, const int32_t* n_tiles_per_layer_host, int band, uint32_t* items_out_host,
                         int64_t capacity);
 XVEC_API int xvec_tdnn_stack(const struct XvecLayerDesc* tdnn_host, int n_tdnn, const void* x_dev, int64_t rows, int64_t x_ld,
diff --git a/speaker-recognition-x-vectors_b200/_lib.py b/speaker-recognition-x-vectors_b200/_lib.py
--- a/speaker-recognition-x-vectors_b200/_lib.py
+++ b/speaker-recognition-x-vectors_b200/_lib.py
@@ -11,7 +11,7 @@
 F32, BF16 = 0, 1
 E_ARG, E_CUDA, E_DEVICE = -1, -2, -3
 TILE_N, POOL_BLOCK, POOL_CHUNK, MAX_TAPS = 256, 128, 128, 8
-ABI_VERSION = 7
+ABI_VERSION = 8
 MAX_STACK = 6
 STACK_MAX_TAP_OFFSET = 8
 
@@ -43,7 +43,7 @@
     "xvec_extract_forward": (c_int, [POINTER(LayerDesc), c_int, c_void_p, c_int64, c_int64, c_void_p, c_void_p, c_int64, c_void_p, c_void_p,
                                      c_void_p, c_void_p, c_int, c_void_p, c_void_p, c_void_p, c_void_p, c_void_p, POINTER(LayerDesc), c_int,
                                      c_void_p, c_void_p, c_int64, c_void_p, c_int64, c_void_p, c_int64, c_void_p]),
-    "xvec_stack_ctrl_bytes": (c_int64, [c_int64, c_int]),
+    "xvec_stack_ctrl_bytes": (c_int64, [c_int64, c_int, c_int]),
     "xvec_stack_plan": (c_int64, [c_int64, c_int, POINTER(c_int32), c_int, c_void_p, c_int64]),
     "xvec_linear_small": (c_int, [c_void_p, c_int, c_int64, c_int, c_int64, c_void_p, c_int, c_int64, c_void_p, c_int, c_void_p, c_int, c_int64,
                                   c_void_p]),
diff --git a/speaker-recognition-x-vectors_b200/build.py b/speaker-recognition-x-vectors_b200/build.py
--- a/speaker-recognition-x-vectors_b200/build.py
+++ b/speaker-recognition-x-vectors_b200/build.py
@@ -8,7 +8,7 @@
 CSRC = os.path.join(HERE, "csrc")
 LIB = os.path.join(HERE, "libxvec_b200.so")
 SOURCES = ["capi.cu", "tdnn_gemm.cu", "tdnn_stack.cu", "fc_small.cu", "pool.cu", "mfcc.cu"]
-HEADERS = ["ptx.cuh", "gemm_tile.cuh", "xvec_internal.h", os.path.join("..", "..", "include", "xvec_b200.h")]
+HEADERS = ["ptx.cuh", "gemm_tile.cuh", "pool_finalize.cuh", "xvec_internal.h", os.path.join("..", "..", "include", "xvec_b200.h")]
 NVCC_FLAGS = ["-gencode", "arch=compute_100a,code=sm_100a", "-O3", "-std=c++17", "-lineinfo", "-Xcompiler", "-fPIC",
               "-Xcompiler", "-fvisibility=hidden", "--expt-relaxed-constexpr"]
 
diff --git a/speaker-recognition-x-vectors_b200/csrc/capi.cu b/speaker-recognition-x-vectors_b200/csrc/capi.cu
--- a/speaker-recognition-x-vectors_b200/csrc/capi.cu
+++ b/speaker-recognition-x-vectors_b200/csrc/capi.cu
@@ -145,7 +145,7 @@
   return gemm_pool(l, x_dev, x_rows, x_ld, rows, row_utt_dev, blk_slot_base_dev, part_dev, stream);
 }
 
-int64_t xvec_stack_ctrl_bytes(int64_t rows, int n_tdnn) { return stack_ctrl_bytes(rows, n_tdnn); }
+int64_t xvec_stack_ctrl_bytes(int64_t rows, int n_tdnn, int n_utts) { return stack_ctrl_bytes(rows, n_tdnn, n_utts); }
 int64_t xvec_stack_plan(int64_t rows, int n_layers, const int32_t* n_tiles_per_layer_host, int band, uint32_t* items_out_host,
                         int64_t capacity) {
   return stack_plan(rows, n_layers, n_tiles_per_layer_host, band, items_out_host, capacity);
@@ -161,14 +161,15 @@
                     int64_t ctrl_bytes, int band, void* stream) {
   if (!tdnn) return set_error(XVEC_E_ARG, "tdnn_host is NULL");
   return stack_dispatch(tdnn, n_tdnn, x_dev, rows, x_ld, act0_dev, act1_dev, act_ld, row_utt_dev, blk_slot_base_dev, part_dev, ctrl_dev,
-                        ctrl_bytes, band, stream);
-}
-
-static int frame_stack(const XvecLayerDesc* tdnn, int n_tdnn, const void* x, int64_t rows, int64_t x_ld, void* act0, void* act1,
-                       int64_t act_ld, const int32_t* row_utt, const int32_t* blk_slot_base, float* part, void* ctrl, int64_t ctrl_bytes,
-                       void* stream) {
+                        ctrl_bytes, band, nullptr, 0, stream);
+}
+
+static int frame_stack_pooled(const XvecLayerDesc* tdnn, int n_tdnn, const void* x, int64_t rows, int64_t x_ld, void* act0, void* act1,
+                              int64_t act_ld, const int32_t* row_utt, const int32_t* blk_slot_base, float* part, const StackFinalize& fin,
+                              int n_utts, void* ctrl, int64_t ctrl_bytes, void* stream) {
   if (ctrl && stack_supported(tdnn, n_tdnn, rows))
-    return stack_dispatch(tdnn, n_tdnn, x, rows, x_ld, act0, act1, act_ld, row_utt, blk_slot_base, part, ctrl, ctrl_bytes, 0, stream);
+    return stack_dispatch(tdnn, n_tdnn, x, rows, x_ld, act0, act1, act_ld, row_utt, blk_slot_base, part, ctrl, ctrl_bytes, 0, &fin, n_utts,
+                          stream);
   void* act[2] = {act0, act1};
   const void* h = x;
   int64_t h_ld = x_ld;
@@ -178,7 +179,10 @@
     h = act[i & 1];
     h_ld = act_ld;
   }
-  return gemm_pool(tdnn[n_tdnn - 1], h, rows, h_ld, rows, row_utt, blk_slot_base, part, stream);
+  const int rc = gemm_pool(tdnn[n_tdnn - 1], h, rows, h_ld, rows, row_utt, blk_slot_base, part, stream);
+  if (rc) return rc;
+  return xvec_pool_finalize(part, fin.utt_slot_start, fin.n_pool, n_utts, tdnn[n_tdnn - 1].n, fin.scale, fin.shift, nullptr, fin.out,
+                            fin.out_lp, XVEC_BF16, fin.lp_ld, stream);
 }
 
 static int segment_head(const XvecLayerDesc* fc, int n_fc, const void* a, int64_t a_ld, int n_utts, void* fc_tmp, void* splitk_ws,
@@ -214,12 +218,12 @@
   if (n_fc == 2 && !fc_tmp_dev) return set_error(XVEC_E_ARG, "fc_tmp_dev is NULL");
   const bool lp_head = n_fc > 0 && fc[0].dtype == XVEC_BF16;
   if (lp_head && !pooled_lp_dev) return set_error(XVEC_E_ARG, "pooled_lp_dev is required for bf16 segment layers");
-  int rc = frame_stack(tdnn, n_tdnn, x_dev, rows, x_ld, act0_dev, act1_dev, act_ld, row_utt_dev, blk_slot_base_dev, part_dev, ctrl_dev,
-                       ctrl_bytes, stream);
-  if (rc) return rc;
+  if (n_utts <= 0 || !utt_slot_start_dev || !n_pool_dev) return set_error(XVEC_E_ARG, "bad utterance layout");
+  if ((bn_last_scale_dev == nullptr) != (bn_last_shift_dev == nullptr)) return set_error(XVEC_E_ARG, "bn_scale and bn_shift must be given together");
   const int64_t pooled_ld = 2 * static_cast<int64_t>(tdnn[n_tdnn - 1].n);
-  rc = xvec_pool_finalize(part_dev, utt_slot_start_dev, n_pool_dev, n_utts, tdnn[n_tdnn - 1].n, bn_last_scale_dev, bn_last_shift_dev, nullptr,
-                          pooled_dev, pooled_lp_dev, XVEC_BF16, pooled_ld, stream);
+  const StackFinalize fin{utt_slot_start_dev, n_pool_dev, bn_last_scale_dev, bn_last_shift_dev, pooled_dev, pooled_lp_dev, pooled_ld, nullptr, 0};
+  int rc = frame_stack_pooled(tdnn, n_tdnn, x_dev, rows, x_ld, act0_dev, act1_dev, act_ld, row_utt_dev, blk_slot_base_dev, part_dev, fin, n_utts,
+                              ctrl_dev, ctrl_bytes, stream);
   if (rc) return rc;
   return segment_head(fc, n_fc, lp_head ? pooled_lp_dev : static_cast<const void*>(pooled_dev), pooled_ld, n_utts, fc_tmp_dev, splitk_ws_dev,
                       splitk_ws_bytes, out_dev, out_ld, stream);
diff --git a/speaker-recognition-x-vectors_b200/csrc/pool.cu b/speaker-recognition-x-vectors_b200/csrc/pool.cu
--- a/speaker-recognition-x-vectors_b200/csrc/pool.cu
+++ b/speaker-recognition-x-vectors_b200/csrc/pool.cu
@@ -1,6 +1,6 @@
 #include <cuda_bf16.h>
 
-#include "xvec_internal.h"
+#include "pool_finalize.cuh"
 
 namespace xvec {
 
@@ -79,59 +79,12 @@
                      const float* __restrict__ scale, const float* __restrict__ shift, const float* __restrict__ pivot,
                      float* __restrict__ out, void* __restrict__ out_lp, int lp_dtype, long long lp_ld) {
   const int u = blockIdx.x;
-  const int col = blockIdx.y * 128 + threadIdx.x;
-  __shared__ double inv_n[2];
-  if (threadIdx.x == 0) {
-    const int n0 = n_rows[u];
-    inv_n[0] = n0 > 0 ? 1.0 / n0 : 0.0;
-    inv_n[1] = n0 > 1 ? 1.0 / (n0 - 1) : 0.0;
-  }
+  const int col[1] = {static_cast<int>(blockIdx.y) * 128 + static_cast<int>(threadIdx.x)};
+  __shared__ double2 inv_n;
+  if (threadIdx.x == 0) inv_n = pool_inv_n(n_rows[u]);
   __syncthreads();
-  if (col >= p) return;
-  const int sl0 = slot_start[u], sl1 = slot_start[u + 1];
-  double S = 0.0, Q = 0.0;
-  int sl = sl0;
-  for (; sl + 4 <= sl1; sl += 4) {
-    float a[4], b[4];
-#pragma unroll
-    for (int i = 0; i < 4; ++i) {
-      const float* src = part + static_cast<size_t>(sl + i) * 2 * p + col;
-      a[i] = src[0];
-      b[i] = src[p];
-    }
-#pragma unroll
-    for (int i = 0; i < 4; ++i) {
-      S += static_cast<double>(a[i]);
-      Q += static_cast<double>(b[i]);
-    }
-  }
-  for (; sl < sl1; ++sl) {
-    const float* src = part + static_cast<size_t>(sl) * 2 * p + col;
-    S += static_cast<double>(src[0]);
-    Q += static_cast<double>(src[p]);
-  }
-  const int n = n_rows[u];
-  const double nan = __longlong_as_double(0x7ff8000000000000LL);
-  const double mean = n > 0 ? S * inv_n[0] + (pivot ? static_cast<double>(pivot[static_cast<size_t>(u) * p + col]) : 0.0) : nan;
-  double var = n > 1 ? (Q - S * S * inv_n[0]) * inv_n[1] : nan;
-  if (var < 0.0) var = 0.0;
-  const float sc = scale ? scale[col] : 1.f;
-  const float sh = shift ? shift[col] : 0.f;
-  const float m = static_cast<float>(mean * sc + sh);
-  const float sd = fabsf(sc) * sqrtf(static_cast<float>(var));
-  out[static_cast<size_t>(u) * 2 * p + col] = m;
-  out[static_cast<size_t>(u) * 2 * p + p + col] = sd;
-  if (out_lp) {
-    if (lp_dtype == XVEC_BF16) {
-      __nv_bfloat16* o = reinterpret_cast<__nv_bfloat16*>(out_lp) + static_cast<size_t>(u) * lp_ld;
-      o[col] = __float2bfloat16_rn(m);
-      o[p + col] = __float2bfloat16_rn(sd);
-    } else {
-      float* o = reinterpret_cast<float*>(out_lp) + static_cast<size_t>(u) * lp_ld;
-      o[col] = m;
-      o[p + col] = sd;
-    }
-  }
+  if (col[0] >= p) return;
+  pool_finalize_cols<1>(part, slot_start[u], slot_start[u + 1], p, col, u, n_rows[u], inv_n, scale, shift, pivot, out, out_lp, lp_dtype, lp_ld);
 }
 
 __global__ void __launch_bounds__(256)
diff --git a/speaker-recognition-x-vectors_b200/csrc/pool_finalize.cuh b/speaker-recognition-x-vectors_b200/csrc/pool_finalize.cuh
--- /dev/null
+++ b/speaker-recognition-x-vectors_b200/csrc/pool_finalize.cuh
@@ -0,0 +1,80 @@
+#pragma once
+#include <cuda_bf16.h>
+
+#include "xvec_internal.h"
+
+namespace xvec {
+
+__device__ __forceinline__ double2 pool_inv_n(int n) { return make_double2(n > 0 ? 1.0 / n : 0.0, n > 1 ? 1.0 / (n - 1) : 0.0); }
+
+template <int NC>
+__device__ __forceinline__ void pool_finalize_cols(const float* part, int sl0, int sl1, int p, const int (&col)[NC], int u, int n, double2 inv_n,
+                                                   const float* scale, const float* shift, const float* pivot, float* out, void* out_lp,
+                                                   int lp_dtype, long long lp_ld) {
+  double S[NC], Q[NC];
+#pragma unroll
+  for (int c = 0; c < NC; ++c) S[c] = Q[c] = 0.0;
+  int sl = sl0;
+  for (; sl + 4 <= sl1; sl += 4) {
+    float a[4][NC], b[4][NC];
+#pragma unroll
+    for (int i = 0; i < 4; ++i) {
+#pragma unroll
+      for (int c = 0; c < NC; ++c) {
+        const float* src = part + static_cast<size_t>(sl + i) * 2 * p + (col[c] < p ? col[c] : 0);
+        a[i][c] = __ldcg(src);
+        b[i][c] = __ldcg(src + p);
+      }
+    }
+#pragma unroll
+    for (int i = 0; i < 4; ++i) {
+#pragma unroll
+      for (int c = 0; c < NC; ++c) {
+        S[c] += static_cast<double>(a[i][c]);
+        Q[c] += static_cast<double>(b[i][c]);
+      }
+    }
+  }
+  for (; sl < sl1; ++sl) {
+    float a[NC], b[NC];
+#pragma unroll
+    for (int c = 0; c < NC; ++c) {
+      const float* src = part + static_cast<size_t>(sl) * 2 * p + (col[c] < p ? col[c] : 0);
+      a[c] = __ldcg(src);
+      b[c] = __ldcg(src + p);
+    }
+#pragma unroll
+    for (int c = 0; c < NC; ++c) {
+      S[c] += static_cast<double>(a[c]);
+      Q[c] += static_cast<double>(b[c]);
+    }
+  }
+  const double nan = __longlong_as_double(0x7ff8000000000000LL);
+#pragma unroll
+  for (int c = 0; c < NC; ++c) {
+    const int cc = col[c];
+    if (cc >= p) continue;
+    const double mean = n > 0 ? S[c] * inv_n.x + (pivot ? static_cast<double>(pivot[static_cast<size_t>(u) * p + cc]) : 0.0) : nan;
+    double var = n > 1 ? (Q[c] - S[c] * S[c] * inv_n.x) * inv_n.y : nan;
+    if (var < 0.0) var = 0.0;
+    const float sc = scale ? scale[cc] : 1.f;
+    const float sh = shift ? shift[cc] : 0.f;
+    const float m = static_cast<float>(mean * sc + sh);
+    const float sd = fabsf(sc) * sqrtf(static_cast<float>(var));
+    out[static_cast<size_t>(u) * 2 * p + cc] = m;
+    out[static_cast<size_t>(u) * 2 * p + p + cc] = sd;
+    if (out_lp) {
+      if (lp_dtype == XVEC_BF16) {
+        __nv_bfloat16* o = reinterpret_cast<__nv_bfloat16*>(out_lp) + static_cast<size_t>(u) * lp_ld;
+        o[cc] = __float2bfloat16_rn(m);
+        o[p + cc] = __float2bfloat16_rn(sd);
+      } else {
+        float* o = reinterpret_cast<float*>(out_lp) + static_cast<size_t>(u) * lp_ld;
+        o[cc] = m;
+        o[p + cc] = sd;
+      }
+    }
+  }
+}
+
+}
diff --git a/speaker-recognition-x-vectors_b200/csrc/ptx.cuh b/speaker-recognition-x-vectors_b200/csrc/ptx.cuh
--- a/speaker-recognition-x-vectors_b200/csrc/ptx.cuh
+++ b/speaker-recognition-x-vectors_b200/csrc/ptx.cuh
@@ -125,6 +125,20 @@
 }
 __device__ __forceinline__ void red_release_gpu_add_u32(uint32_t* p, uint32_t v) {
   asm volatile("red.release.gpu.global.add.u32 [%0], %1;" ::"l"(p), "r"(v) : "memory");
+}
+__device__ __forceinline__ uint32_t atom_add_relaxed_gpu_u32(uint32_t* p, uint32_t v) {
+  uint32_t old;
+  asm volatile("atom.relaxed.gpu.global.add.u32 %0, [%1], %2;" : "=r"(old) : "l"(p), "r"(v) : "memory");
+  return old;
+}
+__device__ __forceinline__ void fence_acq_rel_gpu() { asm volatile("fence.acq_rel.gpu;" ::: "memory"); }
+__device__ __forceinline__ uint32_t ld_acquire_cta_shared_u32(uint32_t smem_addr) {
+  uint32_t v;
+  asm volatile("ld.acquire.cta.shared::cta.u32 %0, [%1];" : "=r"(v) : "r"(smem_addr) : "memory");
+  return v;
+}
+__device__ __forceinline__ void st_release_cta_shared_u32(uint32_t smem_addr, uint32_t v) {
+  asm volatile("st.release.cta.shared::cta.u32 [%0], %1;" ::"r"(smem_addr), "r"(v) : "memory");
 }
 __device__ __forceinline__ uint32_t atom_add_acq_rel_cta_shared_u32(uint32_t smem_addr, uint32_t v) {
   uint32_t old;
diff --git a/speaker-recognition-x-vectors_b200/csrc/tdnn_stack.cu b/speaker-recognition-x-vectors_b200/csrc/tdnn_stack.cu
--- a/speaker-recognition-x-vectors_b200/csrc/tdnn_stack.cu
+++ b/speaker-recognition-x-vectors_b200/csrc/tdnn_stack.cu
@@ -1,4 +1,5 @@
 #include "gemm_tile.cuh"
+#include "pool_finalize.cuh"
 #include <cuda_bf16.h>
 
 #include <mutex>
@@ -26,8 +27,11 @@
 static_assert((EPI_WARPS & (EPI_WARPS - 1)) == 0, "publish() counts the epilogue warps of a CTA modulo EPI_WARPS");
 constexpr int DEP_WARP = 2 + EPI_WARPS;
 constexpr int WPROD_WARP = DEP_WARP + 1;
-constexpr int STACK_THREADS = GEMM_THREADS + 64;
+constexpr int FIN_WARP = WPROD_WARP + 1;
+constexpr int STACK_THREADS = GEMM_THREADS + 96;
+constexpr int FIN_QUEUE = 16;
 constexpr int STACK_MAX_REGS = 112;
+constexpr int STACK_POOL_GROUPS = 2 * 31;
 
 struct StackLayer {
   int n, n_tiles, taps, cpt;
@@ -53,6 +57,7 @@
   const int* row_utt;
   const int* blk_slot_base;
   float* part;
+  StackFinalize fin;
   unsigned long long pol_a, pol_b, pol_y;
   int dbg;
   int runahead;
@@ -228,6 +233,11 @@
   __shared__ uint64_t sfull_bar[SCHED_SLOTS], sempty_bar[SCHED_SLOTS], dep_bar[SCHED_SLOTS], credit_bar[CREDIT_BARS];
   __shared__ uint32_t sched_item[SCHED_SLOTS];
   __shared__ uint32_t pub_cnt[4];
+  __shared__ uint32_t pool_cnt[4];
+  __shared__ int2 pool_rng[4][2];
+  __shared__ int4 fin_rng[FIN_QUEUE];
+  __shared__ int fin_nt[FIN_QUEUE];
+  __shared__ uint32_t fin_seq[FIN_QUEUE], fin_claim, fin_taken, epi_exited;
   __shared__ uint32_t tmem_base_smem;
 
   uint8_t* base = smem_raw + ((1024u - (smem_u32(smem_raw) & 1023u)) & 1023u);
@@ -238,7 +248,9 @@
   const uint32_t rank = cluster_ctarank();
 
   if (warp == 0 && lane == 0) {
-    for (int c = 0; c < 4; ++c) pub_cnt[c] = 0;
+    for (int c = 0; c < 4; ++c) pub_cnt[c] = pool_cnt[c] = 0;
+    for (int c = 0; c < FIN_QUEUE; ++c) fin_seq[c] = 0;
+    fin_claim = fin_taken = epi_exited = 0;
     for (int l = 0; l < p.n_layers; ++l) {
       tma_prefetch_desc(&maps.a[l]);
       tma_prefetch_desc(&maps.b[l]);
@@ -450,6 +462,58 @@
       atomicAdd(p.counter + 1, static_cast<unsigned>(c_spun));
       atomicAdd(p.counter + 2, static_cast<unsigned>(c_polls));
     })
+  } else if (warp == FIN_WARP) {
+    if (p.fin.out) {
+      const StackFinalize& F = p.fin;
+      for (uint32_t idx = 0;; ++idx) {
+        const int q = static_cast<int>(idx % FIN_QUEUE);
+        int4 r = make_int4(0, -1, 0, -1);
+        int nt = 0, state = 0;
+        if (lane == 0) {
+          while (!state) {
+            const uint32_t exited = ld_acquire_cta_shared_u32(smem_u32(&epi_exited));
+            if (ld_acquire_cta_shared_u32(smem_u32(&fin_seq[q])) == idx + 1u) {
+              r = fin_rng[q];
+              nt = fin_nt[q];
+              st_release_cta_shared_u32(smem_u32(&fin_taken), idx + 1u);
+              state = 1;
+            } else if (exited == static_cast<uint32_t>(EPI_WARPS)) {
+              state = 2;
+            } else {
+              __nanosleep(64);
+            }
+          }
+        }
+        __syncwarp();
+        if (__shfl_sync(0xffffffffu, state, 0) == 2) break;
+        r = make_int4(__shfl_sync(0xffffffffu, r.x, 0), __shfl_sync(0xffffffffu, r.y, 0), __shfl_sync(0xffffffffu, r.z, 0),
+                      __shfl_sync(0xffffffffu, r.w, 0));
+        nt = __shfl_sync(0xffffffffu, nt, 0);
+        const int u0 = min(r.x, r.z), u1 = max(r.y, r.w);
+        const int g = 2 * nt + static_cast<int>(rank);
+        const int n_last = p.L[p.n_layers - 1].n;
+        fence_acq_rel_gpu();
+        for (int base = u0; base <= u1; base += 32) {
+          const int u = base + lane;
+          bool done = false;
+          if (u <= u1) {
+            const uint32_t c = (u >= r.x && u <= r.y ? 1u : 0u) + (u >= r.z && u <= r.w ? 1u : 0u);
+            const int slots = __ldg(F.utt_slot_start + u + 1) - __ldg(F.utt_slot_start + u);
+            done = atom_add_relaxed_gpu_u32(F.arrivals + static_cast<size_t>(u) * F.groups + g, c) + c == static_cast<uint32_t>(slots);
+          }
+          uint32_t m = __ballot_sync(0xffffffffu, done);
+          if (m) fence_acq_rel_gpu();
+          while (m) {
+            const int uf = base + __ffs(m) - 1;
+            m &= m - 1;
+            const int col[4] = {g * BN_CTA + lane, g * BN_CTA + 32 + lane, g * BN_CTA + 64 + lane, g * BN_CTA + 96 + lane};
+            const int n = __ldg(F.n_pool + uf);
+            pool_finalize_cols<4>(p.part, __ldg(F.utt_slot_start + uf), __ldg(F.utt_slot_start + uf + 1), n_last, col, uf, n, pool_inv_n(n),
+                                  F.scale, F.shift, nullptr, F.out, F.out_lp, XVEC_BF16, F.lp_ld);
+          }
+        }
+      }
+    }
   } else {
     const int q = warp & 3;
     const int cbeg = ((warp - 2) >> 2) * (BN / 2);
@@ -473,6 +537,32 @@
       pend = nullptr;
     };
     auto flush = [&]() { publish(true); };
+    auto pool_publish = [&](int it, int nt, const PoolPrefetch& pre) {
+      __syncwarp();
+      int lo = 0x7fffffff, hi = -1;
+#pragma unroll
+      for (int k = 0; k < 4; ++k)
+        if (pre.my_u[k] >= 0) {
+          lo = min(lo, pre.my_u[k]);
+          hi = max(hi, pre.my_u[k]);
+        }
+      lo = __reduce_min_sync(0xffffffffu, lo);
+      hi = __reduce_max_sync(0xffffffffu, hi);
+      if (lane == 0) {
+        if ((warp & 3) == 0) pool_rng[it & 3][(warp - 2) >> 2] = make_int2(lo, hi);
+        if ((atom_add_acq_rel_cta_shared_u32(smem_u32(&pool_cnt[it & 3]), 1u) & (EPI_WARPS - 1)) == EPI_WARPS - 1) {
+          const int2 r0 = pool_rng[it & 3][0], r1 = pool_rng[it & 3][1];
+          if (min(r0.x, r1.x) <= max(r0.y, r1.y)) {
+            const uint32_t idx = atomicAdd(&fin_claim, 1u);
+            while (idx - ld_acquire_cta_shared_u32(smem_u32(&fin_taken)) >= static_cast<uint32_t>(FIN_QUEUE)) __nanosleep(32);
+            fin_rng[idx % FIN_QUEUE] = make_int4(r0.x, r0.y, r1.x, r1.y);
+            fin_nt[idx % FIN_QUEUE] = nt;
+            st_release_cta_shared_u32(smem_u32(&fin_seq[idx % FIN_QUEUE]), idx + 1u);
+          }
+        }
+      }
+      __syncwarp();
+    };
     XVEC_CNT(unsigned long long e_wait[2] = {0, 0}, e_busy[2] = {0, 0}, e_tail = 0; long long e_t0 = 0, e_t1 = 0;)
     uint32_t item = ring_read(0);
     for (int it = 0;; ++it) {
@@ -525,6 +615,7 @@
         pool_epilogue_tile_t(pa, pre, tmem_base + buf * BN + (static_cast<uint32_t>(q * 32) << 16) + cbeg, pch, pf0, lane, release_tmem);
         if (!released) release_tmem();
         if (pend) flush();
+        if (p.fin.out) pool_publish(it, nt, pre);
       } else {
         const CUtensorMap* my = &maps.y[layer];
         uint32_t va[32], vb[32];
@@ -590,7 +681,10 @@
       atomicAdd(p.counter + 7, static_cast<unsigned>(e_tail >> 6));
     })
     if (pend) flush();
-    if (lane == 0) tma_store_wait_all();
+    if (lane == 0) {
+      tma_store_wait_all();
+      atom_add_acq_rel_cta_shared_u32(smem_u32(&epi_exited), 1u);
+    }
   }
 
   tc_fence_before();
@@ -659,10 +753,13 @@
   return p.total_items;
 }
 
-int64_t stack_ctrl_bytes(int64_t rows, int n_layers) {
-  if (rows <= 0 || n_layers < 2) return 0;
+static int64_t ctrl_used_bytes(int64_t rows, int n_layers, int n_utts, int groups) {
   const int64_t m_tiles = (rows + BM - 1) / BM;
-  return 256 + (n_layers - 1) * m_tiles * 4;
+  return 256 + (n_layers - 1) * m_tiles * 4 + static_cast<int64_t>(n_utts) * groups * 4;
+}
+int64_t stack_ctrl_bytes(int64_t rows, int n_layers, int n_utts) {
+  if (rows <= 0 || n_layers < 2 || n_utts < 0) return 0;
+  return ctrl_used_bytes(rows, n_layers, n_utts, STACK_POOL_GROUPS);
 }
 
 XVEC_DEFINE_WATCHDOG_BINDER(bind_watchdog_stack)
@@ -774,12 +871,14 @@
 
 int stack_dispatch(const XvecLayerDesc* tdnn, int n_tdnn, const void* x, int64_t rows, int64_t x_ld, void* act0, void* act1,
                    int64_t act_ld, const int32_t* row_utt, const int32_t* blk_slot_base, float* part, void* ctrl, int64_t ctrl_bytes,
-                   int band, void* stream) {
+                   int band, const StackFinalize* fin, int n_utts, void* stream) {
   int rc = device_check();
   if (rc) return rc;
   if (!stack_supported(tdnn, n_tdnn, rows)) return set_error(XVEC_E_ARG, "layer stack is not supported by the fused stack kernel");
   if (!x || !act0 || !act1 || !row_utt || !blk_slot_base || !part || !ctrl) return set_error(XVEC_E_ARG, "null pointer argument");
-  if (ctrl_bytes < stack_ctrl_bytes(rows, n_tdnn) || (reinterpret_cast<uintptr_t>(ctrl) & 127u))
+  if (fin && (n_utts <= 0 || !fin->utt_slot_start || !fin->n_pool || !fin->out)) return set_error(XVEC_E_ARG, "bad pooling finalize arguments");
+  if (!fin) n_utts = 0;
+  if (ctrl_bytes < stack_ctrl_bytes(rows, n_tdnn, n_utts) || (reinterpret_cast<uintptr_t>(ctrl) & 127u))
     return set_error(XVEC_E_ARG, "ctrl_dev must be 128-byte aligned and hold xvec_stack_ctrl_bytes() bytes");
   StackKey key;
   memset(&key, 0, sizeof(key));
@@ -829,6 +928,12 @@
   p.row_utt = row_utt;
   p.blk_slot_base = blk_slot_base;
   p.part = part;
+  const int groups = 2 * p.L[n_tdnn - 1].n_tiles;
+  if (fin) {
+    p.fin = *fin;
+    p.fin.arrivals = p.ready + static_cast<size_t>(n_tdnn - 1) * p.m_tiles;
+    p.fin.groups = groups;
+  }
 #ifdef XVEC_DEBUG
   {
     const char* e = getenv("XVEC_STACK_DBG");
@@ -836,7 +941,7 @@
   }
 #endif
   cudaStream_t st = static_cast<cudaStream_t>(stream);
-  cudaError_t e = cudaMemsetAsync(ctrl, 0, static_cast<size_t>(stack_ctrl_bytes(rows, n_tdnn)), st);
+  cudaError_t e = cudaMemsetAsync(ctrl, 0, static_cast<size_t>(ctrl_used_bytes(rows, n_tdnn, n_utts, groups)), st);
   if (e != cudaSuccess) return set_error(XVEC_E_CUDA, "cudaMemsetAsync(ctrl): %s", cudaGetErrorString(e));
   if (all_tf32)
     return launch_pair<tdnn_stack_kernel<true>>("tdnn_stack_kernel", STACK_THREADS, stack_smem_bytes<true>(), grid, bind_watchdog_stack, st, maps, p);
diff --git a/speaker-recognition-x-vectors_b200/csrc/xvec_internal.h b/speaker-recognition-x-vectors_b200/csrc/xvec_internal.h
--- a/speaker-recognition-x-vectors_b200/csrc/xvec_internal.h
+++ b/speaker-recognition-x-vectors_b200/csrc/xvec_internal.h
@@ -26,12 +26,22 @@
                const float* bn_shift, int relu, void* y, int y_dtype, int64_t y_ld, void* ws, int64_t ws_bytes, void* stream);
 int gemm_pool(const XvecLayerDesc& l, const void* x, int64_t x_rows, int64_t x_ld, int64_t rows, const int32_t* row_utt,
               const int32_t* blk_slot_base, float* part, void* stream);
+struct StackFinalize {
+  const int32_t* utt_slot_start;
+  const int32_t* n_pool;
+  const float *scale, *shift;
+  float* out;
+  void* out_lp;
+  long long lp_ld;
+  unsigned* arrivals;
+  int groups;
+};
 bool stack_supported(const XvecLayerDesc* tdnn, int n_tdnn, int64_t rows);
-int64_t stack_ctrl_bytes(int64_t rows, int n_layers);
+int64_t stack_ctrl_bytes(int64_t rows, int n_layers, int n_utts);
 int64_t stack_plan(int64_t rows, int n_layers, const int32_t* n_tiles_per_layer, int band, uint32_t* items_out, int64_t capacity);
 int stack_dispatch(const XvecLayerDesc* tdnn, int n_tdnn, const void* x, int64_t rows, int64_t x_ld, void* act0, void* act1,
                    int64_t act_ld, const int32_t* row_utt, const int32_t* blk_slot_base, float* part, void* ctrl, int64_t ctrl_bytes,
-                   int band, void* stream);
+                   int band, const StackFinalize* fin, int n_utts, void* stream);
 bool fc_small_supported(int64_t rows, int k, int n, int64_t x_ld, int64_t w_ld, const void* x, const void* w, int dtype);
 int fc_small_dispatch(const void* x, int dtype, int64_t rows, int k, int64_t x_ld, const void* w, int n, int64_t w_ld, const float* bias,
                       int relu, void* y, int y_dtype, int64_t y_ld, void* stream);
diff --git a/speaker-recognition-x-vectors_b200/xvector.py b/speaker-recognition-x-vectors_b200/xvector.py
--- a/speaker-recognition-x-vectors_b200/xvector.py
+++ b/speaker-recognition-x-vectors_b200/xvector.py
@@ -76,13 +76,10 @@
         self.fc_tmp = self.ws = self.ws_for = None
 
     def ensure(self, rows, n_slots, n_utts):
+        grow_ctrl = rows > self.rows_cap or n_utts > self.utts_cap
         if rows > self.rows_cap:
             self.rows_cap = max(rows, int(self.rows_cap * 1.25))
             self.act = [torch.empty((self.rows_cap, self.ld), dtype=self.act_dtype, device=self.device) for _ in range(2)]
-            need = _lib.load().xvec_stack_ctrl_bytes(self.rows_cap, _lib.MAX_STACK)
-            self.ctrl = torch.empty(need + 128, dtype=torch.uint8, device=self.device)
-            off = (-self.ctrl.data_ptr()) % 128
-            self.ctrl = self.ctrl[off: off + need]
         if n_slots > self.slots_cap:
             self.slots_cap = max(n_slots, int(self.slots_cap * 1.25))
             self.part = torch.empty((self.slots_cap, 2, self.pool_dim), dtype=torch.float32, device=self.device)
@@ -92,6 +89,11 @@
             self.pooled_lp = (torch.empty((self.utts_cap, 2 * self.pool_dim), dtype=self.act_dtype, device=self.device)
                               if self.act_dtype != torch.float32 else None)
             self.fc_tmp = None
+        if grow_ctrl:
+            need = _lib.load().xvec_stack_ctrl_bytes(self.rows_cap, _lib.MAX_STACK, self.utts_cap)
+            self.ctrl = torch.empty(need + 128, dtype=torch.uint8, device=self.device)
+            off = (-self.ctrl.data_ptr()) % 128
+            self.ctrl = self.ctrl[off: off + need]
 
     def ensure_head(self, n_utts, fc_shapes, width):
         if self.fc_tmp is None or self.fc_tmp.shape[0] < n_utts or self.fc_tmp.shape[1] != width:
```

Result: slower. 700,700 (median of 6 runs) (-23.3%).
